# filimonov/ClickHouse

Measured on AMD Instinct MI355X. Metric: rows/sec + achieved HBM GB/s, filter+GROUP-BY on 1 B-row Int64 blocks, 1/2/4/8 GPU, higher is better.
Workload: dtype int64; 1 GPU; BASELINE.json configs[1]: SELECT sum(a), count() WHERE a < 214748365 (~10% pass) over Int64 rows, HBM-resident, fused HIP filter+sum kernel; rows_per_gpu=1000000000, parallelism=single GPU

## Files before the change

### clickhouse_amd/csrc/chgpu_internal.h

```cpp
#pragma once

#include <hip/hip_runtime.h>

#include <cstdarg>
#include <cstdint>
#include <cstdio>
#include <cstring>
#include <map>
#include <string>
#include <type_traits>
#include <vector>

#include "../../include/chgpu.h"

typedef uint64_t u64;
typedef int64_t i64;
typedef uint32_t u32;
typedef int32_t i32;
typedef uint8_t u8;
typedef uint16_t u16;
typedef int16_t i16;
typedef int8_t i8;

int chgpu_set_error(int code, const char * fmt, ...);

#define CHGPU_HIP(expr)                                                                                       \
    do                                                                                                        \
    {                                                                                                         \
        hipError_t _e = (expr);                                                                               \
        if (_e != hipSuccess)                                                                                 \
            return chgpu_set_error(_e == hipErrorOutOfMemory ? CHGPU_ERR_OOM : CHGPU_ERR_DEVICE, "%s: %s (%s:%d)", \
                                   #expr, hipGetErrorString(_e), __FILE__, __LINE__);                        \
    } while (0)

#define CHGPU_TRY(expr)      \
    do                       \
    {                        \
        int _rc = (expr);    \
        if (_rc != CHGPU_OK) \
            return _rc;      \
    } while (0)

#define CHGPU_REQUIRE(cond, code, ...)              \
    do                                              \
    {                                               \
        if (!(cond))                                \
            return chgpu_set_error(code, __VA_ARGS__); \
    } while (0)

static constexpr size_t CHGPU_PAD = 64;

struct chgpu_ctx
{
    int device = 0;
    hipStream_t stream = nullptr;
    bool owns_stream = false;
    int num_cus = 256;
    void * scratch = nullptr;
    size_t scratch_bytes = 0;
    void * pinned = nullptr;
    size_t pinned_bytes = 0;
    hipEvent_t ev_start = nullptr, ev_stop = nullptr;
    u64 counters[CHGPU_N_COUNTERS] = {0};
    u32 * crc_lut_dev = nullptr;
    std::multimap<size_t, void *> pool_free;
    size_t pool_cached_bytes = 0;
    size_t pool_limit_bytes = (size_t)96 << 30;
    long refs = 0;
    bool zombie = false;
    hipStream_t copy_stream = nullptr;
    static constexpr int UPLOAD_RING = 32;
    hipEvent_t upload_done[UPLOAD_RING] = {nullptr};
    hipEvent_t upload_gate = nullptr;
    u64 upload_next_ticket = 1;
    std::map<std::string, long long> options;
};

long long chgpu_opt(const chgpu_ctx * ctx, const char * name, long long dflt);

void chgpu_ctx_retain(chgpu_ctx * ctx);
void chgpu_ctx_release(chgpu_ctx * ctx);

struct chgpu_col
{
    chgpu_ctx * ctx = nullptr;
    int type = 0;
    u64 rows = 0;
    void * data = nullptr;
    void * base = nullptr;
    bool owns = false;
    size_t alloc_bytes = 0;
    int * shared_refs = nullptr;
};

struct ChgpuDeviceGuard
{
    int prev = -1;
    bool switched = false;
    explicit ChgpuDeviceGuard(const chgpu_ctx * ctx)
    {
        if (ctx && hipGetDevice(&prev) == hipSuccess && prev != ctx->device)
            switched = hipSetDevice(ctx->device) == hipSuccess;
    }
    ~ChgpuDeviceGuard()
    {
        if (switched)
            (void)hipSetDevice(prev);
    }
    ChgpuDeviceGuard(const ChgpuDeviceGuard &) = delete;
    ChgpuDeviceGuard & operator=(const ChgpuDeviceGuard &) = delete;
};

static inline size_t chgpu_type_size(int type)
{
    switch (type)
    {
        case CHGPU_I64: case CHGPU_U64: case CHGPU_F64: return 8;
        case CHGPU_U32: case CHGPU_I32: case CHGPU_F32: return 4;
        case CHGPU_U16: case CHGPU_I16: return 2;
        case CHGPU_U8: case CHGPU_I8: return 1;
        default: return 0;
    }
}

static inline bool chgpu_type_is_float(int type) { return type == CHGPU_F64 || type == CHGPU_F32; }
static inline bool chgpu_type_is_int(int type) { return !chgpu_type_is_float(type) && chgpu_type_size(type) != 0; }
static inline bool chgpu_type_is_signed(int type) { return type == CHGPU_I64 || type == CHGPU_I32 || type == CHGPU_I16 || type == CHGPU_I8; }
static inline int chgpu_sum_result_type(int t)
{
    if (chgpu_type_is_float(t)) return CHGPU_F64;
    return chgpu_type_is_signed(t) ? CHGPU_I64 : CHGPU_U64;
}

int chgpu_scratch(chgpu_ctx * ctx, size_t bytes, void ** out);
int chgpu_pool_alloc(chgpu_ctx * ctx, size_t bytes, void ** out, size_t * class_bytes);
void chgpu_pool_free(chgpu_ctx * ctx, void * p, size_t class_bytes);
int chgpu_pinned(chgpu_ctx * ctx, size_t bytes, void ** out);
int chgpu_col_new(chgpu_ctx * ctx, int type, u64 rows, chgpu_col ** out);
int chgpu_read_back(chgpu_ctx * ctx, const void * dev, void * host, size_t bytes);
int chgpu_crc_lut(chgpu_ctx * ctx, const u32 ** lut_dev);

static inline u32 chgpu_grid_for(chgpu_ctx * ctx, u64 work_items, u32 block, u32 blocks_per_cu = 8)
{
    u64 want = (work_items + block - 1) / block;
    u64 cap = (u64)ctx->num_cus * blocks_per_cu;
    if (want < 1) want = 1;
    return (u32)(want < cap ? want : cap);
}

int chgpu_scan_exclusive_u32_u64(chgpu_ctx * ctx, const u32 * in, u64 * out, u64 n, u64 * total_dev, void * tmp, size_t tmp_bytes);
int chgpu_scan_inclusive_u32_u64(chgpu_ctx * ctx, const u32 * in, u64 * out, u64 n, u64 * total_dev, void * tmp, size_t tmp_bytes);
size_t chgpu_scan_tmp_bytes(u64 n);
int chgpu_partition_by_key_byte(chgpu_ctx * ctx, const chgpu_col * keys, u32 shift, u32 n_cols, const chgpu_col * const * cols, chgpu_col ** outs);
int chgpu_partition_core(chgpu_ctx * ctx, const u32 * sel, u64 n, u32 num_shards, u32 n_cols, const chgpu_col * const * cols, chgpu_col ** outs, u64 * counts);
int str_validate_offsets(chgpu_ctx * ctx, const chgpu_col * offsets_u64, const chgpu_col * chars_u8);

template <typename F>
static void dispatch_width(size_t bytes, F && fn)
{
    switch (bytes)
    {
        case 8: return fn(u64{});
        case 4: return fn(u32{});
        case 2: return fn(u16{});
        default: return fn(u8{});
    }
}

template <int LO, int HI, typename F>
static void dispatch_const(u32 v, F && fn)
{
    if constexpr (LO < HI)
        if (v > (u32)LO)
            return dispatch_const<LO + 1, HI>(v, fn);
    fn(std::integral_constant<int, LO>{});
}

template <u32... CODES>
struct OneOf
{
    static bool has(u32 v) { return ((v == CODES) || ...); }
    template <typename F>
    static bool dispatch(u32 v, F && fn)
    {
        return ((v == CODES ? (fn(std::integral_constant<u32, CODES>{}), true) : false) || ...);
    }
};

#ifdef __HIPCC__

static constexpr int WAVE = 64;

__device__ __forceinline__ u32 lane_id() { return __builtin_amdgcn_mbcnt_hi(~0u, __builtin_amdgcn_mbcnt_lo(~0u, 0u)); }

__device__ __forceinline__ u32 mbcnt(u64 mask)
{
    return __builtin_amdgcn_mbcnt_hi((u32)(mask >> 32), __builtin_amdgcn_mbcnt_lo((u32)mask, 0u));
}

__device__ __forceinline__ u64 shfl_down_u64(u64 v, int delta)
{
    u32 lo = __shfl_down((u32)v, delta, WAVE);
    u32 hi = __shfl_down((u32)(v >> 32), delta, WAVE);
    return ((u64)hi << 32) | lo;
}

__device__ __forceinline__ u64 wave_reduce_add_u64(u64 v)
{
#pragma unroll
    for (int d = 32; d >= 1; d >>= 1)
        v += shfl_down_u64(v, d);
    return v;
}

__device__ __forceinline__ double wave_reduce_add_f64(double v)
{
#pragma unroll
    for (int d = 32; d >= 1; d >>= 1)
        v += __longlong_as_double((long long)shfl_down_u64((u64)__double_as_longlong(v), d));
    return v;
}

__device__ __forceinline__ u32 wave_reduce_add_u32(u32 v)
{
#pragma unroll
    for (int d = 32; d >= 1; d >>= 1)
        v += __shfl_down(v, d, WAVE);
    return v;
}

__device__ __forceinline__ u64 wave_reduce_max_u64(u64 v)
{
#pragma unroll
    for (int d = 32; d >= 1; d >>= 1)
    {
        const u64 o = shfl_down_u64(v, d);
        v = o > v ? o : v;
    }
    return v;
}

__device__ __host__ __forceinline__ u64 agg_order_key(u64 bits, int type)
{
    switch (type)
    {
        case CHGPU_I64: case CHGPU_I32: case CHGPU_I16: case CHGPU_I8: return bits ^ 0x8000000000000000ull;
        case CHGPU_F64: case CHGPU_F32: return (bits >> 63) ? ~bits : bits ^ 0x8000000000000000ull;
        default: return bits;
    }
}
__device__ __host__ __forceinline__ u64 agg_order_key_inverse(u64 key, int type)
{
    switch (type)
    {
        case CHGPU_I64: case CHGPU_I32: case CHGPU_I16: case CHGPU_I8: return key ^ 0x8000000000000000ull;
        case CHGPU_F64: case CHGPU_F32: return (key >> 63) ? key ^ 0x8000000000000000ull : ~key;
        default: return key;
    }
}

__device__ __forceinline__ u64 dev_intHash64(u64 x)
{
    x ^= x >> 33;
    x *= 0xff51afd7ed558ccdULL;
    x ^= x >> 33;
    x *= 0xc4ceb9fe1a85ec53ULL;
    x ^= x >> 33;
    return x;
}

__device__ __forceinline__ u32 dev_crc32c_tab(const u32 * __restrict__ lut, u64 x)
{
    u32 r = 0;
#pragma unroll
    for (int j = 0; j < 8; ++j)
        r ^= lut[j * 256 + ((x >> (8 * j)) & 0xFF)];
    return r;
}

__device__ __forceinline__ u32 dev_crc32c_zero8(u32 crc)
{
#pragma unroll 1
    for (int k = 0; k < 64; ++k)
        crc = (crc >> 1) ^ (0x82F63B78u & (0u - (crc & 1u)));
    return crc;
}

#endif
```

### clickhouse_amd/csrc/core.hip

```cpp
#include "chgpu_internal.h"

#include <mutex>

static thread_local char g_last_error[512] = "";

int chgpu_set_error(int code, const char * fmt, ...)
{
    va_list ap;
    va_start(ap, fmt);
    vsnprintf(g_last_error, sizeof(g_last_error), fmt, ap);
    va_end(ap);
    return code;
}

extern "C" const char * chgpu_last_error(void) { return g_last_error; }
extern "C" int chgpu_abi_version(void) { return CHGPU_ABI_VERSION; }

extern "C" int chgpu_ctx_create(int device_id, void * hip_stream, chgpu_ctx ** out)
{
    CHGPU_REQUIRE(out, CHGPU_ERR_BAD_ARGUMENTS, "chgpu_ctx_create: out is NULL");
    int n_dev = 0;
    CHGPU_HIP(hipGetDeviceCount(&n_dev));
    CHGPU_REQUIRE(device_id >= 0 && device_id < n_dev, CHGPU_ERR_BAD_ARGUMENTS, "device %d out of range (%d devices)", device_id, n_dev);
    chgpu_ctx probe_dev;
    probe_dev.device = device_id;
    ChgpuDeviceGuard guard(&probe_dev);
    hipDeviceProp_t prop;
    CHGPU_HIP(hipGetDeviceProperties(&prop, device_id));
    chgpu_ctx * ctx = new chgpu_ctx();
    ctx->device = device_id;
    ctx->num_cus = prop.multiProcessorCount > 0 ? prop.multiProcessorCount : 256;
    if (hip_stream)
    {
        ctx->stream = (hipStream_t)hip_stream;
        ctx->owns_stream = false;
    }
    else
    {
        hipError_t e = hipStreamCreateWithFlags(&ctx->stream, hipStreamNonBlocking);
        if (e != hipSuccess)
        {
            delete ctx;
            return chgpu_set_error(CHGPU_ERR_DEVICE, "hipStreamCreate: %s", hipGetErrorString(e));
        }
        ctx->owns_stream = true;
    }
    (void)hipEventCreate(&ctx->ev_start);
    (void)hipEventCreate(&ctx->ev_stop);
    *out = ctx;
    return CHGPU_OK;
}

static void ctx_teardown(chgpu_ctx * ctx)
{
    ChgpuDeviceGuard guard(ctx);
    (void)hipStreamSynchronize(ctx->stream);
    if (ctx->copy_stream)
    {
        (void)hipStreamSynchronize(ctx->copy_stream);
        (void)hipStreamDestroy(ctx->copy_stream);
    }
    for (auto & e : ctx->upload_done)
        if (e) (void)hipEventDestroy(e);
    if (ctx->upload_gate) (void)hipEventDestroy(ctx->upload_gate);
    if (ctx->scratch) (void)hipFree(ctx->scratch);
    for (auto & kv : ctx->pool_free)
        (void)hipFree(kv.second);
    ctx->pool_free.clear();
    if (ctx->pinned) (void)hipHostFree(ctx->pinned);
    if (ctx->crc_lut_dev) (void)hipFree(ctx->crc_lut_dev);
    if (ctx->ev_start) (void)hipEventDestroy(ctx->ev_start);
    if (ctx->ev_stop) (void)hipEventDestroy(ctx->ev_stop);
    if (ctx->owns_stream) (void)hipStreamDestroy(ctx->stream);
    delete ctx;
}

void chgpu_ctx_retain(chgpu_ctx * ctx)
{
    if (ctx)
        ++ctx->refs;
}

void chgpu_ctx_release(chgpu_ctx * ctx)
{
    if (ctx && --ctx->refs == 0 && ctx->zombie)
        ctx_teardown(ctx);
}

extern "C" int chgpu_ctx_destroy(chgpu_ctx * ctx)
{
    if (!ctx)
        return CHGPU_OK;
    if (ctx->refs > 0)
    {
        ctx->zombie = true;
        return CHGPU_OK;
    }
    ctx_teardown(ctx);
    return CHGPU_OK;
}

extern "C" int chgpu_ctx_synchronize(chgpu_ctx * ctx)
{
    ChgpuDeviceGuard _dev_guard(ctx);
    CHGPU_REQUIRE(ctx, CHGPU_ERR_BAD_ARGUMENTS, "ctx is NULL");
    CHGPU_HIP(hipStreamSynchronize(ctx->stream));
    return CHGPU_OK;
}

static std::mutex g_opt_mu;
static std::map<std::string, long long> g_opt_defaults;
static const char * const CHGPU_OPTION_NAMES[] = {
    "agg_no_partition", "debug", "deterministic_float_sums", "test_chain_grid", "test_group_array_fail_alloc", "test_keydict_chunk_rows", "test_keydict_weak_tags", "test_limit_by_fail_alloc", "test_limit_by_grid", "test_quantile_fail_alloc", "test_quantile_hist_budget",
    "test_string_fail_alloc", "test_uniq_fail_growth",
    "tune_agg_lds_threads", "tune_agg_no_ranged", "tune_agg_ranged_s", "tune_cmp_wg", "tune_expr_wg", "tune_exprn_wg", "tune_fcount_wg",
    "tune_filter_no_multi", "tune_fs2_wg", "tune_fs_wg", "tune_fscatter_wg", "tune_gb_kib", "tune_gb_no_tiled",
    "tune_gb_no_word_passes", "tune_gb_no_two_level", "tune_gb_nocnt32", "tune_gb_noops", "tune_gb_nowide", "tune_gb_s", "tune_gb_tile",
    "tune_gb_unitdiv", "tune_jit_unroll", "tune_jit_wg_map", "tune_jit_wg_sum", "tune_join_cap_shift", "tune_join_eager_build",
    "tune_join_lds_min_rows", "tune_join_no_dense_prefilter", "tune_join_no_fused_payload", "tune_join_no_lds_filter",
    "tune_join_no_lds_probe", "tune_join_no_prefilter", "tune_join_no_dense_map", "tune_join_no_radix",
    "tune_join_no_regions", "tune_join_no_slice_build", "tune_join_region_kib", "tune_join_region_min_rows", "tune_quantile_hist_rounds", "tune_quantile_no_lds_scatter", "tune_str_contains_general",
};

long long chgpu_opt(const chgpu_ctx * ctx, const char * name, long long dflt)
{
    if (ctx && !ctx->options.empty())
    {
        auto it = ctx->options.find(name);
        if (it != ctx->options.end())
            return it->second;
    }
    std::lock_guard<std::mutex> lk(g_opt_mu);
    if (g_opt_defaults.empty())
        return dflt;
    auto it = g_opt_defaults.find(name);
    return it != g_opt_defaults.end() ? it->second : dflt;
}

extern "C" int chgpu_ctx_set_option(chgpu_ctx * ctx, const char * name, int64_t value)
{
    CHGPU_REQUIRE(name, CHGPU_ERR_BAD_ARGUMENTS, "NULL argument");
    bool known = false;
    for (const char * n : CHGPU_OPTION_NAMES)
        known = known || strcmp(n, name) == 0;
    CHGPU_REQUIRE(known, CHGPU_ERR_BAD_ARGUMENTS, "unknown option '%s'", name);
    if (ctx)
        ctx->options[name] = value;
    else
    {
        std::lock_guard<std::mutex> lk(g_opt_mu);
        g_opt_defaults[name] = value;
    }
    return CHGPU_OK;
}

extern "C" int chgpu_ctx_trim(chgpu_ctx * ctx)
{
    ChgpuDeviceGuard _dev_guard(ctx);
    CHGPU_REQUIRE(ctx, CHGPU_ERR_BAD_ARGUMENTS, "ctx is NULL");
    CHGPU_HIP(hipStreamSynchronize(ctx->stream));
    for (auto & kv : ctx->pool_free)
        (void)hipFree(kv.second);
    ctx->pool_free.clear();
    ctx->pool_cached_bytes = 0;
    if (ctx->scratch)
        (void)hipFree(ctx->scratch);
    ctx->scratch = nullptr;
    ctx->scratch_bytes = 0;
    return CHGPU_OK;
}

extern "C" int chgpu_ctx_counters(chgpu_ctx * ctx, uint64_t out[CHGPU_N_COUNTERS])
{
    ChgpuDeviceGuard _dev_guard(ctx);
    CHGPU_REQUIRE(ctx && out, CHGPU_ERR_BAD_ARGUMENTS, "NULL argument");
    memcpy(out, ctx->counters, sizeof(ctx->counters));
    return CHGPU_OK;
}

extern "C" int chgpu_timer_start(chgpu_ctx * ctx)
{
    ChgpuDeviceGuard _dev_guard(ctx);
    CHGPU_REQUIRE(ctx, CHGPU_ERR_BAD_ARGUMENTS, "ctx is NULL");
    CHGPU_HIP(hipEventRecord(ctx->ev_start, ctx->stream));
    return CHGPU_OK;
}

extern "C" int chgpu_timer_stop_ms(chgpu_ctx * ctx, double * elapsed_ms)
{
    ChgpuDeviceGuard _dev_guard(ctx);
    CHGPU_REQUIRE(ctx && elapsed_ms, CHGPU_ERR_BAD_ARGUMENTS, "NULL argument");
    CHGPU_HIP(hipEventRecord(ctx->ev_stop, ctx->stream));
    CHGPU_HIP(hipEventSynchronize(ctx->ev_stop));
    float ms = 0;
    CHGPU_HIP(hipEventElapsedTime(&ms, ctx->ev_start, ctx->ev_stop));
    *elapsed_ms = ms;
    return CHGPU_OK;
}

int chgpu_scratch(chgpu_ctx * ctx, size_t bytes, void ** out)
{
    if (bytes > ctx->scratch_bytes)
    {
        ChgpuDeviceGuard guard(ctx);
        CHGPU_HIP(hipStreamSynchronize(ctx->stream));
        if (ctx->scratch)
            CHGPU_HIP(hipFree(ctx->scratch));
        ctx->scratch = nullptr;
        ctx->scratch_bytes = 0;
        size_t want = bytes + bytes / 4 + (1 << 20);
        CHGPU_HIP(hipMalloc(&ctx->scratch, want));
        ctx->scratch_bytes = want;
    }
    *out = ctx->scratch;
    return CHGPU_OK;
}

int chgpu_pinned(chgpu_ctx * ctx, size_t bytes, void ** out)
{
    if (bytes > ctx->pinned_bytes)
    {
        ChgpuDeviceGuard guard(ctx);
        CHGPU_HIP(hipStreamSynchronize(ctx->stream));
        if (ctx->pinned)
            CHGPU_HIP(hipHostFree(ctx->pinned));
        ctx->pinned = nullptr;
        ctx->pinned_bytes = 0;
        size_t want = bytes < 4096 ? 4096 : bytes;
        CHGPU_HIP(hipHostMalloc(&ctx->pinned, want, hipHostMallocDefault));
        ctx->pinned_bytes = want;
    }
    *out = ctx->pinned;
    return CHGPU_OK;
}

int chgpu_read_back(chgpu_ctx * ctx, const void * dev, void * host, size_t bytes)
{
    void * stage = nullptr;
    CHGPU_TRY(chgpu_pinned(ctx, bytes, &stage));
    CHGPU_HIP(hipMemcpyAsync(stage, dev, bytes, hipMemcpyDeviceToHost, ctx->stream));
    CHGPU_HIP(hipStreamSynchronize(ctx->stream));
    memcpy(host, stage, bytes);
    return CHGPU_OK;
}

static size_t pool_class(size_t bytes)
{
    if (bytes < 4096)
        return 4096;
    size_t p = 4096;
    while (p * 2 <= bytes)
        p *= 2;
    for (int q = 4; q <= 8; ++q)
        if (p / 4 * q >= bytes)
            return p / 4 * q;
    return p * 2;
}

int chgpu_pool_alloc(chgpu_ctx * ctx, size_t bytes, void ** out, size_t * class_bytes)
{
    const size_t cls = pool_class(bytes);
    ChgpuDeviceGuard guard(ctx);
    auto it = ctx->pool_free.lower_bound(cls);
    if (it != ctx->pool_free.end() && it->first <= cls + cls / 2)
    {
        *out = it->second;
        *class_bytes = it->first;
        ctx->pool_cached_bytes -= it->first;
        ctx->pool_free.erase(it);
        return CHGPU_OK;
    }
    hipError_t e = hipMalloc(out, cls);
    if (e == hipErrorOutOfMemory && !ctx->pool_free.empty())
    {
        (void)hipGetLastError();
        (void)hipStreamSynchronize(ctx->stream);
        for (auto & kv : ctx->pool_free)
            (void)hipFree(kv.second);
        ctx->pool_free.clear();
        ctx->pool_cached_bytes = 0;
        e = hipMalloc(out, cls);
    }
    if (e != hipSuccess)
        return chgpu_set_error(e == hipErrorOutOfMemory ? CHGPU_ERR_OOM : CHGPU_ERR_DEVICE, "hipMalloc(%zu): %s", cls, hipGetErrorString(e));
    *class_bytes = cls;
    return CHGPU_OK;
}

void chgpu_pool_free(chgpu_ctx * ctx, void * p, size_t class_bytes)
{
    if (!p)
        return;
    if (ctx->pool_cached_bytes + class_bytes > ctx->pool_limit_bytes)
    {
        (void)hipFree(p);
        return;
    }
    ctx->pool_free.emplace(class_bytes, p);
    ctx->pool_cached_bytes += class_bytes;
}

int chgpu_col_new(chgpu_ctx * ctx, int type, u64 rows, chgpu_col ** out)
{
    size_t es = chgpu_type_size(type);
    CHGPU_REQUIRE(es, CHGPU_ERR_BAD_ARGUMENTS, "unknown column type %d", type);
    ChgpuDeviceGuard guard(ctx);
    size_t bytes = rows * es + 2 * CHGPU_PAD;
    void * base = nullptr;
    size_t cls = 0;
    CHGPU_TRY(chgpu_pool_alloc(ctx, bytes, &base, &cls));
    chgpu_col * c = new chgpu_col();
    chgpu_ctx_retain(ctx);
    c->ctx = ctx;
    c->type = type;
    c->rows = rows;
    c->base = base;
    c->data = (char *)base + CHGPU_PAD;
    c->owns = true;
    c->alloc_bytes = cls;
    *out = c;
    return CHGPU_OK;
}

extern "C" int chgpu_col_alloc(chgpu_ctx * ctx, int type, uint64_t rows, chgpu_col ** out)
{
    ChgpuDeviceGuard _dev_guard(ctx);
    CHGPU_REQUIRE(ctx && out, CHGPU_ERR_BAD_ARGUMENTS, "NULL argument");
    return chgpu_col_new(ctx, type, rows, out);
}

extern "C" int chgpu_col_upload(chgpu_ctx * ctx, int type, const void * host_ptr, uint64_t rows, chgpu_col ** out)
{
    ChgpuDeviceGuard _dev_guard(ctx);
    CHGPU_REQUIRE(ctx && out && (host_ptr || rows == 0), CHGPU_ERR_BAD_ARGUMENTS, "NULL argument");
    chgpu_col * c = nullptr;
    CHGPU_TRY(chgpu_col_new(ctx, type, rows, &c));
    if (rows)
    {
        hipError_t e = hipMemcpyAsync(c->data, host_ptr, rows * chgpu_type_size(type), hipMemcpyHostToDevice, ctx->stream);
        if (e == hipSuccess)
            e = hipStreamSynchronize(ctx->stream);
        if (e != hipSuccess)
        {
            chgpu_col_free(c);
            return chgpu_set_error(CHGPU_ERR_DEVICE, "upload: %s", hipGetErrorString(e));
        }
    }
    *out = c;
    return CHGPU_OK;
}

extern "C" int chgpu_host_alloc(size_t bytes, void ** out)
{
    CHGPU_REQUIRE(out, CHGPU_ERR_BAD_ARGUMENTS, "NULL argument");
    CHGPU_HIP(hipHostMalloc(out, bytes ? bytes : 1, hipHostMallocDefault));
    return CHGPU_OK;
}

extern "C" int chgpu_host_free(void * p)
{
    if (p)
        CHGPU_HIP(hipHostFree(p));
    return CHGPU_OK;
}

extern "C" int chgpu_col_upload_async(chgpu_ctx * ctx, int type, const void * pinned_host_ptr, uint64_t rows, chgpu_col ** out, uint64_t * ticket_out)
{
    CHGPU_REQUIRE(ctx && out && ticket_out && (pinned_host_ptr || rows == 0), CHGPU_ERR_BAD_ARGUMENTS, "NULL argument");
    ChgpuDeviceGuard guard(ctx);
    if (!ctx->copy_stream)
    {
        CHGPU_HIP(hipStreamCreateWithFlags(&ctx->copy_stream, hipStreamNonBlocking));
        CHGPU_HIP(hipEventCreateWithFlags(&ctx->upload_gate, hipEventDisableTiming));
        for (auto & e : ctx->upload_done)
            CHGPU_HIP(hipEventCreateWithFlags(&e, hipEventDisableTiming));
    }
    chgpu_col * c = nullptr;
    CHGPU_TRY(chgpu_col_new(ctx, type, rows, &c));
    const u64 ticket = ctx->upload_next_ticket++;
    hipEvent_t done = ctx->upload_done[ticket % chgpu_ctx::UPLOAD_RING];
    hipError_t e = hipSuccess;
    if ((e = hipEventRecord(ctx->upload_gate, ctx->stream)) == hipSuccess && (e = hipStreamWaitEvent(ctx->copy_stream, ctx->upload_gate, 0)) == hipSuccess)
    {
        if (rows)
            e = hipMemcpyAsync(c->data, pinned_host_ptr, rows * chgpu_type_size(type), hipMemcpyHostToDevice, ctx->copy_stream);
        if (e == hipSuccess)
            e = hipEventRecord(done, ctx->copy_stream);
        if (e == hipSuccess)
            e = hipStreamWaitEvent(ctx->stream, done, 0);
    }
    if (e != hipSuccess)
    {
        chgpu_col_free(c);
        return chgpu_set_error(CHGPU_ERR_DEVICE, "upload_async: %s", hipGetErrorString(e));
    }
    *out = c;
    *ticket_out = ticket;
    return CHGPU_OK;
}

extern "C" int chgpu_upload_wait(chgpu_ctx * ctx, uint64_t ticket)
{
    ChgpuDeviceGuard _dev_guard(ctx);
    CHGPU_REQUIRE(ctx, CHGPU_ERR_BAD_ARGUMENTS, "ctx is NULL");
    if (ticket == 0 || ticket >= ctx->upload_next_ticket)
        return ticket == 0 ? CHGPU_OK : chgpu_set_error(CHGPU_ERR_BAD_ARGUMENTS, "upload ticket %llu was never issued", (unsigned long long)ticket);
    ChgpuDeviceGuard guard(ctx);
    if (ticket + chgpu_ctx::UPLOAD_RING <= ctx->upload_next_ticket)
    {
        CHGPU_HIP(hipStreamSynchronize(ctx->copy_stream));
        return CHGPU_OK;
    }
    CHGPU_HIP(hipEventSynchronize(ctx->upload_done[ticket % chgpu_ctx::UPLOAD_RING]));
    return CHGPU_OK;
}

extern "C" int chgpu_col_wrap(chgpu_ctx * ctx, int type, void * device_ptr, uint64_t rows, chgpu_col ** out)
{
    ChgpuDeviceGuard _dev_guard(ctx);
    CHGPU_REQUIRE(ctx && out && (device_ptr || rows == 0), CHGPU_ERR_BAD_ARGUMENTS, "NULL argument");
    CHGPU_REQUIRE(chgpu_type_size(type), CHGPU_ERR_BAD_ARGUMENTS, "unknown column type %d", type);
    CHGPU_REQUIRE(((uintptr_t)device_ptr % chgpu_type_size(type)) == 0, CHGPU_ERR_BAD_ARGUMENTS, "device pointer not element-aligned");
    chgpu_col * c = new chgpu_col();
    chgpu_ctx_retain(ctx);
    c->ctx = ctx;
    c->type = type;
    c->rows = rows;
    c->data = device_ptr;
    c->owns = false;
    *out = c;
    return CHGPU_OK;
}

extern "C" int chgpu_col_slice(chgpu_ctx * ctx, const chgpu_col * col, uint64_t start, uint64_t rows, chgpu_col ** out)
{
    ChgpuDeviceGuard _dev_guard(ctx);
    CHGPU_REQUIRE(ctx && col && out, CHGPU_ERR_BAD_ARGUMENTS, "NULL argument");
    CHGPU_REQUIRE(start <= col->rows && rows <= col->rows - start, CHGPU_ERR_BAD_ARGUMENTS,
                  "cut(%llu,%llu) out of bounds of a column of %llu rows", (unsigned long long)start, (unsigned long long)rows, (unsigned long long)col->rows);
    return chgpu_col_wrap(ctx, col->type, (char *)col->data + start * chgpu_type_size(col->type), rows, out);
}

extern "C" int chgpu_col_concat(chgpu_ctx * ctx, uint32_t n, const chgpu_col * const * cols, chgpu_col ** out)
{
    ChgpuDeviceGuard _dev_guard(ctx);
    CHGPU_REQUIRE(ctx && cols && out && n >= 1, CHGPU_ERR_BAD_ARGUMENTS, "NULL argument");
    u64 total = 0;
    for (u32 k = 0; k < n; ++k)
    {
        CHGPU_REQUIRE(cols[k], CHGPU_ERR_BAD_ARGUMENTS, "column %u is NULL", k);
        CHGPU_REQUIRE(cols[k]->type == cols[0]->type, CHGPU_ERR_BAD_ARGUMENTS, "columns of different types cannot be concatenated");
        total += cols[k]->rows;
    }
    chgpu_col * r = nullptr;
    CHGPU_TRY(chgpu_col_new(ctx, cols[0]->type, total, &r));
    const size_t es = chgpu_type_size(cols[0]->type);
    u64 pos = 0;
    for (u32 k = 0; k < n; ++k)
    {
        if (cols[k]->rows)
        {
            hipError_t e = hipMemcpyAsync((char *)r->data + pos * es, cols[k]->data, cols[k]->rows * es, hipMemcpyDeviceToDevice, ctx->stream);
            if (e != hipSuccess)
            {
                chgpu_col_free(r);
                return chgpu_set_error(CHGPU_ERR_DEVICE, "concat copy: %s", hipGetErrorString(e));
            }
        }
        pos += cols[k]->rows;
    }
    *out = r;
    return CHGPU_OK;
}

extern "C" int chgpu_col_download(chgpu_ctx * ctx, const chgpu_col * col, void * host_ptr, uint64_t rows)
{
    ChgpuDeviceGuard _dev_guard(ctx);
    CHGPU_REQUIRE(ctx && col && (host_ptr || rows == 0), CHGPU_ERR_BAD_ARGUMENTS, "NULL argument");
    CHGPU_REQUIRE(rows <= col->rows, CHGPU_ERR_SIZES_MISMATCH, "download of %llu rows from a column of %llu", (unsigned long long)rows, (unsigned long long)col->rows);
    if (rows)
    {
        CHGPU_HIP(hipMemcpyAsync(host_ptr, col->data, rows * chgpu_type_size(col->type), hipMemcpyDeviceToHost, ctx->stream));
        CHGPU_HIP(hipStreamSynchronize(ctx->stream));
    }
    return CHGPU_OK;
}

extern "C" int chgpu_col_download_many(chgpu_ctx * ctx, uint32_t n, const chgpu_col * const * cols, void * const * host_ptrs)
{
    ChgpuDeviceGuard _dev_guard(ctx);
    CHGPU_REQUIRE(ctx && (n == 0 || (cols && host_ptrs)), CHGPU_ERR_BAD_ARGUMENTS, "NULL argument");
    bool any = false;
    for (u32 c = 0; c < n; ++c)
    {
        CHGPU_REQUIRE(cols[c] && (host_ptrs[c] || cols[c]->rows == 0), CHGPU_ERR_BAD_ARGUMENTS, "NULL column or host buffer %u", c);
        if (cols[c]->rows)
        {
            CHGPU_HIP(hipMemcpyAsync(host_ptrs[c], cols[c]->data, cols[c]->rows * chgpu_type_size(cols[c]->type), hipMemcpyDeviceToHost, ctx->stream));
            any = true;
        }
    }
    if (any)
        CHGPU_HIP(hipStreamSynchronize(ctx->stream));
    return CHGPU_OK;
}

extern "C" uint64_t chgpu_col_rows(const chgpu_col * col) { return col ? col->rows : 0; }
extern "C" int chgpu_col_type(const chgpu_col * col) { return col ? col->type : -1; }
extern "C" void * chgpu_col_device_ptr(const chgpu_col * col) { return col ? col->data : nullptr; }

extern "C" int chgpu_col_free(chgpu_col * col)
{
    if (!col)
        return CHGPU_OK;
    if (col->owns && col->base)
    {
        bool last = true;
        if (col->shared_refs)
        {
            last = --*col->shared_refs == 0;
            if (last)
                delete col->shared_refs;
        }
        if (last)
        {
            if (col->alloc_bytes && col->ctx)
                chgpu_pool_free(col->ctx, col->base, col->alloc_bytes);
            else
                (void)hipFree(col->base);
        }
    }
    chgpu_ctx * ctx = col->ctx;
    delete col;
    chgpu_ctx_release(ctx);
    return CHGPU_OK;
}

int chgpu_crc_lut(chgpu_ctx * ctx, const u32 ** lut_dev)
{
    if (!ctx->crc_lut_dev)
    {
        ChgpuDeviceGuard guard(ctx);
        std::vector<u32> lut(8 * 256 + 1);
        auto soft = [](u64 x, u32 crc) {
            for (int i = 0; i < 8; ++i)
            {
                crc ^= (u32)((x >> (8 * i)) & 0xFF);
                for (int k = 0; k < 8; ++k)
                    crc = (crc >> 1) ^ (0x82F63B78u & (0u - (crc & 1u)));
            }
            return crc;
        };
        for (int j = 0; j < 8; ++j)
            for (int b = 0; b < 256; ++b)
                lut[j * 256 + b] = soft((u64)b << (8 * j), 0);
        lut[2048] = soft(0, 0xFFFFFFFFu);
        CHGPU_HIP(hipMalloc((void **)&ctx->crc_lut_dev, lut.size() * sizeof(u32)));
        CHGPU_HIP(hipMemcpyAsync(ctx->crc_lut_dev, lut.data(), lut.size() * sizeof(u32), hipMemcpyHostToDevice, ctx->stream));
        CHGPU_HIP(hipStreamSynchronize(ctx->stream));
    }
    *lut_dev = ctx->crc_lut_dev;
    return CHGPU_OK;
}
```

### clickhouse_amd/csrc/expr_jit.hip

```cpp
#include "chgpu_internal.h"

#include <dlfcn.h>

#include <mutex>
#include <string>

namespace
{

struct Rtc
{
    void * h = nullptr;
    int (*create)(void **, const char *, const char *, int, const char * const *, const char * const *) = nullptr;
    int (*compile)(void *, int, const char * const *) = nullptr;
    int (*log_size)(void *, size_t *) = nullptr;
    int (*log)(void *, char *) = nullptr;
    int (*code_size)(void *, size_t *) = nullptr;
    int (*code)(void *, char *) = nullptr;
    int (*destroy)(void **) = nullptr;
};
Rtc g_rtc;
std::mutex g_jit_mutex;
std::map<std::string, std::vector<char>> g_code_cache;
std::map<std::pair<int, std::string>, hipModule_t> g_module_cache;

int rtc_load()
{
    if (g_rtc.h)
        return CHGPU_OK;
    const char * names[] = {"libhiprtc.so.7", "libhiprtc.so", "/opt/rocm/lib/libhiprtc.so"};
    void * h = nullptr;
    for (const char * n : names)
        if ((h = dlopen(n, RTLD_NOW | RTLD_LOCAL)))
            break;
    if (!h)
        return chgpu_set_error(CHGPU_ERR_NOT_IMPLEMENTED, "cannot load libhiprtc (%s): expressions stay on the CPU", dlerror());
#define SYM(field, name)                                              \
    *(void **)&g_rtc.field = dlsym(h, name);                          \
    if (!g_rtc.field)                                                 \
        return chgpu_set_error(CHGPU_ERR_DEVICE, "libhiprtc lacks %s", name);
    SYM(create, "hiprtcCreateProgram")
    SYM(compile, "hiprtcCompileProgram")
    SYM(log_size, "hiprtcGetProgramLogSize")
    SYM(log, "hiprtcGetProgramLog")
    SYM(code_size, "hiprtcGetCodeSize")
    SYM(code, "hiprtcGetCode")
    SYM(destroy, "hiprtcDestroyProgram")
#undef SYM
    g_rtc.h = h;
    return CHGPU_OK;
}

const char * ctype(int t)
{
    switch (t)
    {
        case CHGPU_I64: return "i64";
        case CHGPU_U64: return "u64";
        case CHGPU_I32: return "i32";
        case CHGPU_U32: return "u32";
        case CHGPU_I16: return "i16";
        case CHGPU_U16: return "u16";
        case CHGPU_I8: return "i8";
        case CHGPU_U8: return "u8";
        case CHGPU_F64: return "f64";
        case CHGPU_F32: return "f32";
        default: return nullptr;
    }
}

int construct(bool sgn, bool flt, size_t size)
{
    if (flt)
        return size == 8 ? CHGPU_F64 : size == 4 ? CHGPU_F32 : -1;
    switch (size)
    {
        case 1: return sgn ? CHGPU_I8 : CHGPU_U8;
        case 2: return sgn ? CHGPU_I16 : CHGPU_U16;
        case 4: return sgn ? CHGPU_I32 : CHGPU_U32;
        case 8: return sgn ? CHGPU_I64 : CHGPU_U64;
        default: return -1;
    }
}
size_t next_size(size_t s) { return s < 8 ? s * 2 : s; }
bool is_sgn(int t) { return chgpu_type_is_signed(t) || chgpu_type_is_float(t); }

struct FnRow;
struct Operands
{
    int rt;
    int t[3];
    std::string n[3];
};
typedef int (*TypeRule)(const FnRow & f, int fn, int a, int b, int c);
typedef std::string (*Emitter)(const Operands & x);
typedef const char * (*Gate)(const chgpu_expr_node * nodes, const chgpu_expr_node & nd, const int * at);

struct FnRow
{
    int code, n_codes;
    int arity;
    TypeRule type;
    int result;
    const char * text;
    const char * text_float;
    Emitter emit;
    Gate gate;
};

int ty_fixed(const FnRow & f, int, int a, int b, int)
{
    return chgpu_type_size(a) && (f.arity < 2 || chgpu_type_size(b)) ? f.result : -1;
}
int ty_date(const FnRow & f, int, int a, int, int) { return a == CHGPU_U16 ? f.result : -1; }
bool both_int(int a, int b) { return chgpu_type_is_int(a) && chgpu_type_is_int(b); }
int ty_add_mul(const FnRow &, int, int a, int b, int)
{
    const size_t sa = chgpu_type_size(a), sb = chgpu_type_size(b);
    return (sa && sb) ? construct(is_sgn(a) || is_sgn(b), chgpu_type_is_float(a) || chgpu_type_is_float(b), next_size(sa > sb ? sa : sb)) : -1;
}
int ty_minus(const FnRow &, int, int a, int b, int)
{
    const size_t sa = chgpu_type_size(a), sb = chgpu_type_size(b);
    return (sa && sb) ? construct(true, chgpu_type_is_float(a) || chgpu_type_is_float(b), next_size(sa > sb ? sa : sb)) : -1;
}
int ty_negate(const FnRow &, int, int a, int, int)
{
    const size_t sa = chgpu_type_size(a);
    return sa ? construct(true, chgpu_type_is_float(a), is_sgn(a) ? sa : next_size(sa)) : -1;
}
int ty_bit(const FnRow &, int, int a, int b, int)
{
    return both_int(a, b) ? construct(is_sgn(a) || is_sgn(b), false, std::max(chgpu_type_size(a), chgpu_type_size(b))) : -1;
}
int ty_int_div(const FnRow &, int, int a, int b, int)
{
    return both_int(a, b) ? construct(is_sgn(a) || is_sgn(b), false, chgpu_type_size(a)) : -1;
}
int ty_modulo(const FnRow &, int, int a, int b, int)
{
    return both_int(a, b) ? construct(is_sgn(a), false, is_sgn(a) ? next_size(chgpu_type_size(b)) : chgpu_type_size(b)) : -1;
}
int ty_if(const FnRow &, int, int a, int b, int c)
{
    const size_t sb = chgpu_type_size(b), sc = chgpu_type_size(c);
    if (!chgpu_type_is_int(a) || !sb || !sc)
        return -1;
    if (b == c)
        return b;
    const bool fb = chgpu_type_is_float(b), fc = chgpu_type_is_float(c);
    const bool has_float = fb || fc, has_integer = !fb || !fc, has_signed = is_sgn(b) || is_sgn(c), has_unsigned = !is_sgn(b) || !is_sgn(c);
    const size_t max_u = std::max(is_sgn(b) ? (size_t)0 : sb, is_sgn(c) ? (size_t)0 : sc);
    const size_t max_s = std::max(is_sgn(b) ? sb : (size_t)0, is_sgn(c) ? sc : (size_t)0);
    const size_t max_i = std::max(fb ? (size_t)0 : sb, fc ? (size_t)0 : sc);
    const size_t max_f = std::max(fb ? sb : (size_t)0, fc ? sc : (size_t)0);
    const size_t m = std::max(sb, sc);
    const bool dbl = (has_float && has_integer && max_i >= max_f) || (has_signed && has_unsigned && max_u >= max_s);
    return construct(has_signed, has_float, dbl ? m * 2 : m);
}
int ty_cast(const FnRow & f, int fn, int a, int, int)
{
    const int to = fn - f.code;
    if (!chgpu_type_size(a) || !chgpu_type_size(to))
        return -1;
    if (chgpu_type_is_float(a) && !chgpu_type_is_float(to))
        return -1;
    return to;
}

const char * const NO_SAFE_DIVISOR = "intDiv / modulo need a constant integer divisor that cannot raise ILLEGAL_DIVISION";
bool constant_divisor(const chgpu_expr_node * nodes, const chgpu_expr_node & nd, const int * at, u64 * bits, u64 * mask)
{
    const chgpu_expr_node & dn = nodes[nd.args[1]];
    if (dn.kind != CHGPU_EX_CONST || !both_int(at[0], at[1]))
        return false;
    const size_t sb = chgpu_type_size(at[1]);
    *mask = sb == 8 ? ~0ull : ((1ull << (8 * sb)) - 1);
    *bits = dn.bits & *mask;
    return *bits != 0;
}
const char * gate_int_div(const chgpu_expr_node * nodes, const chgpu_expr_node & nd, const int * at)
{
    u64 bits = 0, mask = 0;
    if (!constant_divisor(nodes, nd, at, &bits, &mask))
        return NO_SAFE_DIVISOR;
    const bool cast_to_signed = chgpu_type_is_signed(at[0]) && chgpu_type_size(at[0]) <= chgpu_type_size(at[1]);
    return bits == mask && (chgpu_type_is_signed(at[1]) || cast_to_signed) ? NO_SAFE_DIVISOR : nullptr;
}
const char * gate_modulo(const chgpu_expr_node * nodes, const chgpu_expr_node & nd, const int * at)
{
    u64 bits = 0, mask = 0;
    if (!constant_divisor(nodes, nd, at, &bits, &mask))
        return NO_SAFE_DIVISOR;
    if (!chgpu_type_is_signed(at[1]))
        return nullptr;
    return bits == mask || bits == (mask >> 1) + 1 ? NO_SAFE_DIVISOR : nullptr;
}

std::string wide(int t, const std::string & e)
{
    if (chgpu_type_is_float(t))
        return "(f64)" + e;
    return (chgpu_type_is_signed(t) ? "(i64)" : "(u64)") + e;
}

std::string subst(const std::string & text, const Operands & x)
{
    std::string s;
    for (size_t i = 0; i < text.size(); ++i)
    {
        if (text[i] != '$')
            s += text[i];
        else if (text[++i] == 'T')
            s += ctype(x.rt);
        else if (text[i] == 'W')
        {
            ++i;
            s += wide(x.t[text[i] - '0'], x.n[text[i] - '0']);
        }
        else
            s += x.n[text[i] - '0'];
    }
    return s;
}

std::string emit_int_div(const Operands & x)
{
    const int ta = x.t[0], tb = x.t[1];
    if (!chgpu_type_is_signed(ta) && !chgpu_type_is_signed(tb))
        return subst("($T)($0 / $1)", x);
    const int sa_t = construct(true, false, chgpu_type_size(ta));
    const int sb_t = chgpu_type_size(ta) <= chgpu_type_size(tb) ? construct(true, false, chgpu_type_size(tb)) : sa_t;
    return subst(std::string("($T)((") + ctype(sa_t) + ")$0 / (" + ctype(sb_t) + ")$1)", x);
}

const FnRow FUNCTIONS[] = {
    {CHGPU_FN_EQUALS, 1, 2, ty_fixed, CHGPU_U8, "(u8)(eq_($W0, $W1))"},
    {CHGPU_FN_NOT_EQUALS, 1, 2, ty_fixed, CHGPU_U8, "(u8)(!eq_($W0, $W1))"},
    {CHGPU_FN_LESS, 1, 2, ty_fixed, CHGPU_U8, "(u8)(lt_($W0, $W1))"},
    {CHGPU_FN_GREATER, 1, 2, ty_fixed, CHGPU_U8, "(u8)(lt_($W1, $W0))"},
    {CHGPU_FN_LESS_OR_EQUALS, 1, 2, ty_fixed, CHGPU_U8, "(u8)(le_($W0, $W1))"},
    {CHGPU_FN_GREATER_OR_EQUALS, 1, 2, ty_fixed, CHGPU_U8, "(u8)(ge_($W0, $W1))"},
    {CHGPU_FN_PLUS, 1, 2, ty_add_mul, -1, "($T)((u64)$0 + (u64)$1)", "(f64)$0 + (f64)$1"},
    {CHGPU_FN_MINUS, 1, 2, ty_minus, -1, "($T)((u64)$0 - (u64)$1)", "(f64)$0 - (f64)$1"},
    {CHGPU_FN_MULTIPLY, 1, 2, ty_add_mul, -1, "($T)((u64)$0 * (u64)$1)", "(f64)$0 * (f64)$1"},
    {CHGPU_FN_DIVIDE, 1, 2, ty_fixed, CHGPU_F64, "(f64)$0 / (f64)$1"},
    {CHGPU_FN_NEGATE, 1, 1, ty_negate, -1, "($T)(0ull - (u64)$0)", "-$0"},
    {CHGPU_FN_INT_DIV, 1, 2, ty_int_div, -1, nullptr, nullptr, emit_int_div, gate_int_div},
    {CHGPU_FN_MODULO, 1, 2, ty_modulo, -1, "($T)($0 % $1)", nullptr, nullptr, gate_modulo},
    {CHGPU_FN_AND, 1, 2, ty_fixed, CHGPU_U8, "(u8)(($0 != 0) & ($1 != 0))"},
    {CHGPU_FN_OR, 1, 2, ty_fixed, CHGPU_U8, "(u8)(($0 != 0) | ($1 != 0))"},
    {CHGPU_FN_XOR, 1, 2, ty_fixed, CHGPU_U8, "(u8)(($0 != 0) ^ ($1 != 0))"},
    {CHGPU_FN_NOT, 1, 1, ty_fixed, CHGPU_U8, "(u8)!($0 != 0)"},
    {CHGPU_FN_IF, 1, 3, ty_if, -1, "($0 != 0) ? ($T)$1 : ($T)$2"},
    {CHGPU_FN_BIT_AND, 1, 2, ty_bit, -1, "($T)((u64)$0 & (u64)$1)"},
    {CHGPU_FN_BIT_OR, 1, 2, ty_bit, -1, "($T)((u64)$0 | (u64)$1)"},
    {CHGPU_FN_BIT_XOR, 1, 2, ty_bit, -1, "($T)((u64)$0 ^ (u64)$1)"},
    {CHGPU_FN_TO_YEAR, 1, 1, ty_date, CHGPU_U16, "(u16)civil_($0).y"},
    {CHGPU_FN_TO_MONTH, 1, 1, ty_date, CHGPU_U8, "(u8)civil_($0).m"},
    {CHGPU_FN_TO_DAY_OF_MONTH, 1, 1, ty_date, CHGPU_U8, "(u8)civil_($0).d"},
    {CHGPU_FN_TO_YYYYMM, 1, 1, ty_date, CHGPU_U32, "(u32)(civil_($0).y * 100u + civil_($0).m)"},
    {CHGPU_FN_TO_YYYYMMDD, 1, 1, ty_date, CHGPU_U32, "(u32)(civil_($0).y * 10000u + civil_($0).m * 100u + civil_($0).d)"},
    {CHGPU_FN_TO_DAY_OF_WEEK, 1, 1, ty_date, CHGPU_U8, "(u8)(((u32)$0 + 3u) % 7u + 1u)"},
    {CHGPU_FN_TO_QUARTER, 1, 1, ty_date, CHGPU_U8, "(u8)((civil_($0).m - 1u) / 3u + 1u)"},
    {CHGPU_FN_TO_START_OF_MONTH, 1, 1, ty_date, CHGPU_U16, "(u16)((u32)$0 - (civil_($0).d - 1u))"},
    {CHGPU_FN_CAST, 16, 1, ty_cast, -1, "($T)$0"},
};

const FnRow * fn_row(int fn)
{
    for (const FnRow & f : FUNCTIONS)
        if (fn >= f.code && fn < f.code + f.n_codes)
            return &f;
    return nullptr;
}

const char * PRELUDE = R"SRC(
typedef unsigned long long u64; typedef long long i64; typedef unsigned int u32; typedef int i32;
typedef unsigned short u16; typedef short i16; typedef unsigned char u8; typedef signed char i8;
typedef float f32; typedef double f64;
#define DEV static __device__ __forceinline__
// accurate::lessOp / equalsOp (AccurateComparison.h:20-204) on operands widened to i64 / u64 / f64: mathematically exact
DEV bool nan_(i64) { return false; }
DEV bool nan_(u64) { return false; }
DEV bool nan_(f64 x) { return x != x; }
DEV bool lt_(i64 a, i64 b) { return a < b; }
DEV bool lt_(u64 a, u64 b) { return a < b; }
DEV bool lt_(f64 a, f64 b) { return a < b; }
DEV bool lt_(i64 a, u64 b) { return a < 0 || (u64)a < b; }
DEV bool lt_(u64 a, i64 b) { return b >= 0 && a < (u64)b; }
DEV bool lt_(i64 a, f64 b)
{
    if (b != b) return false;
    if (b >= 9223372036854775808.0) return true;
    if (b < -9223372036854775808.0) return false;
    const i64 t = (i64)b; // truncation, exact in range
    if (a != t) return a < t;
    return b - (f64)t > 0;
}
DEV bool lt_(f64 a, i64 b)
{
    if (a != a) return false;
    if (a >= 9223372036854775808.0) return false;
    if (a < -9223372036854775808.0) return true;
    const i64 t = (i64)a;
    if (t != b) return t < b;
    return a - (f64)t < 0;
}
DEV bool lt_(u64 a, f64 b)
{
    if (b != b) return false;
    if (b >= 18446744073709551616.0) return true;
    if (b <= 0) return false;
    const u64 t = (u64)b;
    if (a != t) return a < t;
    return b - (f64)t > 0;
}
DEV bool lt_(f64 a, u64 b)
{
    if (a != a) return false;
    if (a >= 18446744073709551616.0) return false;
    if (a < 0) return true;
    const u64 t = (u64)a;
    if (t != b) return t < b;
    return a - (f64)t < 0;
}
DEV bool eq_(i64 a, i64 b) { return a == b; }
DEV bool eq_(u64 a, u64 b) { return a == b; }
DEV bool eq_(f64 a, f64 b) { return a == b; }
DEV bool eq_(i64 a, u64 b) { return a >= 0 && (u64)a == b; }
DEV bool eq_(u64 a, i64 b) { return b >= 0 && a == (u64)b; }
DEV bool eq_(i64 a, f64 b)
{
    if (!(b >= -9223372036854775808.0 && b < 9223372036854775808.0)) return false;
    const i64 t = (i64)b;
    return t == a && (f64)t == b;
}
DEV bool eq_(f64 a, i64 b) { return eq_(b, a); }
DEV bool eq_(u64 a, f64 b)
{
    if (!(b >= 0 && b < 18446744073709551616.0)) return false;
    const u64 t = (u64)b;
    return t == a && (f64)t == b;
}
DEV bool eq_(f64 a, u64 b) { return eq_(b, a); }
template <typename A, typename B> DEV bool le_(A a, B b) { return !nan_(a) && !nan_(b) && !lt_(b, a); }
template <typename A, typename B> DEV bool ge_(A a, B b) { return !nan_(a) && !nan_(b) && !lt_(a, b); }
// DayNum -> civil date (proleptic Gregorian; what DateLUTImpl's day table holds for DayNum, Common/DateLUTImpl.h)
struct Civil { u32 y, m, d; };
DEV Civil civil_(u32 days)
{
    const u32 z = days + 719468u;
    const u32 era = z / 146097u;
    const u32 doe = z - era * 146097u;
    const u32 yoe = (doe - doe / 1460u + doe / 36524u - doe / 146096u) / 365u;
    const u32 doy = doe - (365u * yoe + yoe / 4u - yoe / 100u);
    const u32 mp = (5u * doy + 2u) / 153u;
    Civil c;
    c.d = doy - (153u * mp + 2u) / 5u + 1u;
    c.m = mp < 10u ? mp + 3u : mp - 9u;
    c.y = yoe + era * 400u + (c.m <= 2u ? 1u : 0u);
    return c;
}
)SRC";

}

struct chgpu_expr
{
    std::vector<chgpu_expr_node> nodes;
    std::vector<int> types;
    std::vector<int> input_types;
    std::string body;
};


namespace
{

int build_body(chgpu_expr * e)
{
    std::string s;
    char buf[256];
    for (size_t k = 0; k < e->nodes.size(); ++k)
    {
        const chgpu_expr_node & nd = e->nodes[k];
        const int t = e->types[k];
        const char * ct = ctype(t);
        std::string rhs;
        if (nd.kind == CHGPU_EX_INPUT)
            rhs = "r.c" + std::to_string(nd.code);
        else if (nd.kind == CHGPU_EX_CONST)
        {
            if (t == CHGPU_F64)
                snprintf(buf, sizeof(buf), "__longlong_as_double((long long)0x%llxull)", (unsigned long long)nd.bits);
            else if (t == CHGPU_F32)
                snprintf(buf, sizeof(buf), "__uint_as_float(0x%xu)", (unsigned)(nd.bits & 0xffffffffu));
            else
                snprintf(buf, sizeof(buf), "(%s)0x%llxull", ct, (unsigned long long)nd.bits);
            rhs = buf;
        }
        else
        {
            const FnRow & f = *fn_row(nd.code);
            Operands x;
            x.rt = t;
            for (int j = 0; j < f.arity; ++j)
            {
                x.t[j] = e->types[nd.args[j]];
                x.n[j] = "n" + std::to_string(nd.args[j]);
            }
            rhs = f.emit ? f.emit(x) : subst(f.text_float && chgpu_type_is_float(t) ? f.text_float : f.text, x);
        }
        s += std::string("    const ") + ct + " n" + std::to_string(k) + " = " + rhs + ";\n";
    }
    e->body = s;
    return CHGPU_OK;
}

u32 vec_rows(const std::vector<int> & types)
{
    size_t wmax = 1, wmin = 8;
    for (int t : types)
    {
        const size_t w = chgpu_type_size(t);
        wmax = std::max(wmax, w);
        wmin = std::min(wmin, w);
    }
    u32 v = (u32)std::max((size_t)16 / wmax, (size_t)4 / wmin);
    return v < 1 ? 1 : v > 16 ? 16 : v;
}

enum Form
{
    FORM_MAP,
    FORM_SUM,
    FORM_WHERE_MAP,
};

struct KernelSpec
{
    Form form = FORM_MAP;
    std::vector<u32> out_nodes;
    int filter_node = -1;
    int value_node = -1;
    u32 vec = 1;
};

static int jit_env(const chgpu_ctx * ctx, const char * name, int dflt) { return (int)chgpu_opt(ctx, name, dflt); }
static int jit_unroll()
{
    static const int v = jit_env(nullptr, "tune_jit_unroll", 4);
    return v;
}
#define JIT_UNROLL jit_unroll()
constexpr u32 JIT_MAX_COLS = 8;

struct JitArgs
{
    const void * in[JIT_MAX_COLS];
    void * out[JIT_MAX_COLS];
    u64 n;
    u64 * part;
    u32 n_parts;
    u32 pad;
};
const char * const ARGS_DECL = "struct Args { const void * in[8]; void * out[8]; u64 n; u64 * part; u32 n_parts; u32 pad; };\n";
static_assert(JIT_MAX_COLS == 8 && sizeof(JitArgs) == 2 * 8 * 8 + 8 + 8 + 4 + 4, "ARGS_DECL restates JitArgs");

struct ResField
{
    std::string type, name, value;
};

std::vector<ResField> out_fields(const chgpu_expr * e, const std::vector<u32> & out_nodes)
{
    std::vector<ResField> fields;
    for (size_t o = 0; o < out_nodes.size(); ++o)
        fields.push_back({ctype(e->types[out_nodes[o]]), "o" + std::to_string(o), "n" + std::to_string(out_nodes[o])});
    return fields;
}

std::string gen_frame(const chgpu_expr * e, const std::string & decls, bool keep, int filter_node, const std::vector<ResField> & fields)
{
    std::string s = PRELUDE + decls + ARGS_DECL + "struct Row {";
    for (size_t j = 0; j < e->input_types.size(); ++j)
        if (e->input_types[j] >= 0)
            s += std::string(" ") + ctype(e->input_types[j]) + " c" + std::to_string(j) + ";";
    s += " };\nstruct Res {";
    if (keep)
        s += " bool keep;";
    for (const ResField & f : fields)
        s += " " + f.type + " " + f.name + ";";
    s += " };\nDEV void eval(const Row & r, Res & o)\n{\n" + e->body;
    if (keep)
        s += filter_node >= 0 ? "    o.keep = n" + std::to_string(filter_node) + " != 0;\n" : std::string("    o.keep = true;\n");
    for (const ResField & f : fields)
        s += "    o." + f.name + " = " + f.value + ";\n";
    return s + "}\n";
}

std::string row_load(const chgpu_expr * e, const std::string & indent, const std::string & index)
{
    std::string s;
    for (size_t j = 0; j < e->input_types.size(); ++j)
        if (e->input_types[j] >= 0)
            s += indent + "r.c" + std::to_string(j) + " = ((const " + ctype(e->input_types[j]) + " *)a.in[" + std::to_string(j) + "])[" + index + "];\n";
    return s;
}

std::string out_store(const std::string & indent, const std::string & type, size_t o, const std::string & index, const std::string & value)
{
    return indent + "((" + type + " *)a.out[" + std::to_string(o) + "])[" + index + "] = " + value + ";\n";
}

std::string gen_source(const chgpu_expr * e, const KernelSpec & ks)
{
    const bool fsum = ks.form == FORM_SUM;
    const u32 V = ks.vec;
    auto vtype = [&](int t) { return std::string("v") + ctype(t) + "_t"; };
    auto otype = [&](size_t o) { return e->types[ks.out_nodes[o]]; };
    const size_t n_out = ks.out_nodes.size();
    std::string vdefs;
    for (int t = 0; t <= CHGPU_F32; ++t)
        vdefs += std::string("typedef ") + ctype(t) + " " + vtype(t) + " __attribute__((ext_vector_type(" + std::to_string(V) + ")));\n";
    std::vector<ResField> fields = out_fields(e, ks.out_nodes);
    if (fsum && ks.value_node >= 0)
        fields.push_back({ctype(e->types[ks.value_node]), "val", "n" + std::to_string(ks.value_node)});
    std::string s = gen_frame(e, vdefs, fsum, ks.filter_node, fields);

    const bool facc = fsum && ks.value_node >= 0 && chgpu_type_is_float(e->types[ks.value_node]);
    auto accumulate = [&](const std::string & indent) {
        std::string t;
        if (ks.value_node >= 0)
            t += indent + (facc ? "acc += o.keep ? (f64)o.val : 0.0;\n" : "acc += o.keep ? (u64)o.val : 0ull;\n");
        return t + indent + "cnt += o.keep ? 1u : 0u;\n";
    };
    const std::string U = std::to_string(JIT_UNROLL), VS = std::to_string(V);
    s += "extern \"C\" __global__ __launch_bounds__(256) void k_run(Args a)\n{\n";
    if (fsum)
        s += facc ? "    f64 acc = 0; u64 cnt = 0;\n" : "    u64 acc = 0; u64 cnt = 0;\n";
    s += "    const u64 nvec = a.n / " + VS + ";\n    constexpr u64 CH = 256ull * " + U + ";\n    const u64 nch = nvec / CH;\n";
    const bool tr_ok = !fsum && V * (u32)JIT_UNROLL == 16;
    std::vector<int> tr_slot(n_out, -1);
    int n_tr = 0;
    if (tr_ok)
        for (size_t o = 0; o < n_out; ++o)
            if (chgpu_type_size(otype(o)) == 1)
                tr_slot[o] = n_tr++;
    if (n_tr)
        s += "    typedef u8 v16b_t __attribute__((ext_vector_type(16)));\n    __shared__ __attribute__((aligned(16))) u8 tr[" + std::to_string(n_tr) + "][4][1024];\n";
    s += "    for (u64 ch = blockIdx.x; ch < nch; ch += gridDim.x)\n    {\n        const u64 sb = ch * CH + (u64)(threadIdx.x >> 6) * (64 * " + U +
         ");\n        const u64 vb = sb + (threadIdx.x & 63);\n";
    for (size_t j = 0; j < e->input_types.size(); ++j)
        if (e->input_types[j] >= 0)
        {
            const std::string vt = vtype(e->input_types[j]), J = std::to_string(j);
            s += "        " + vt + " x" + J + "[" + U + "];\n";
            s += "#pragma unroll\n        for (int k = 0; k < " + U + "; ++k) x" + J + "[k] = __builtin_nontemporal_load((const " + vt + " *)a.in[" + J + "] + vb + (u64)k * 64);\n";
        }
    s += "#pragma unroll\n        for (int k = 0; k < " + U + "; ++k)\n        {\n";
    for (size_t o = 0; o < n_out; ++o)
        s += "            " + vtype(otype(o)) + " y" + std::to_string(o) + ";\n";
    s += "#pragma unroll\n            for (int q = 0; q < " + VS + "; ++q)\n            {\n                Row r; Res o;\n";
    for (size_t j = 0; j < e->input_types.size(); ++j)
        if (e->input_types[j] >= 0)
            s += "                r.c" + std::to_string(j) + " = x" + std::to_string(j) + "[k][q];\n";
    s += "                eval(r, o);\n";
    if (fsum)
        s += accumulate("                ");
    for (size_t o = 0; o < n_out; ++o)
        s += "                y" + std::to_string(o) + "[q] = o.o" + std::to_string(o) + ";\n";
    s += "            }\n";
    for (size_t o = 0; o < n_out; ++o)
    {
        if (tr_slot[o] >= 0)
            s += "            *(" + vtype(otype(o)) + " *)&tr[" + std::to_string(tr_slot[o]) + "][threadIdx.x >> 6][(k * 64 + (threadIdx.x & 63)) * " + VS +
                 "] = y" + std::to_string(o) + ";\n";
        else
            s += out_store("            ", vtype(otype(o)), o, "vb + (u64)k * 64", "y" + std::to_string(o));
    }
    s += "        }\n";
    if (n_tr)
    {
        s += "        __builtin_amdgcn_wave_barrier();\n";
        for (size_t o = 0; o < n_out; ++o)
            if (tr_slot[o] >= 0)
                s += "        *((v16b_t *)((u8 *)a.out[" + std::to_string(o) + "] + sb * " + VS + ") + (threadIdx.x & 63)) = *(const v16b_t *)&tr[" +
                     std::to_string(tr_slot[o]) + "][threadIdx.x >> 6][(threadIdx.x & 63) * 16];\n";
        s += "        __builtin_amdgcn_wave_barrier();\n";
    }
    s += "    }\n";
    s += "    for (u64 i = nch * CH * " + VS + " + (u64)blockIdx.x * 256 + threadIdx.x; i < a.n; i += (u64)gridDim.x * 256)\n    {\n        Row r; Res o;\n";
    s += row_load(e, "        ", "i") + "        eval(r, o);\n";
    if (fsum)
        s += accumulate("        ");
    for (size_t o = 0; o < n_out; ++o)
        s += out_store("        ", ctype(otype(o)), o, "i", "o.o" + std::to_string(o));
    s += "    }\n";
    if (fsum)
    {
        s += R"SRC(
    __shared__ u64 sh_a[4], sh_c[4];
    u64 ab = ACC_BITS(acc);
#pragma unroll
    for (int d = 32; d >= 1; d >>= 1)
    {
        const u64 oa = ((u64)__shfl_down((u32)(ab >> 32), d, 64) << 32) | __shfl_down((u32)ab, d, 64);
        const u64 oc = ((u64)__shfl_down((u32)(cnt >> 32), d, 64) << 32) | __shfl_down((u32)cnt, d, 64);
        ab = ACC_ADD(ab, oa);
        cnt += oc;
    }
    if ((threadIdx.x & 63) == 0) { sh_a[threadIdx.x >> 6] = ab; sh_c[threadIdx.x >> 6] = cnt; }
    __syncthreads();
    if (threadIdx.x == 0)
    {
        u64 ta = sh_a[0], tc = sh_c[0];
        for (int w = 1; w < 4; ++w) { ta = ACC_ADD(ta, sh_a[w]); tc += sh_c[w]; }
        a.part[2 * blockIdx.x] = ta;
        a.part[2 * blockIdx.x + 1] = tc;
    }
}
extern "C" __global__ __launch_bounds__(64) void k_fin(Args a)
{
    if (threadIdx.x != 0) return;
    u64 ta = ACC_ZERO, tc = 0;
    for (u32 p = 0; p < a.n_parts; ++p) { ta = ACC_ADD(ta, a.part[2 * p]); tc += a.part[2 * p + 1]; }
    a.part[2 * a.n_parts] = ta;
    a.part[2 * a.n_parts + 1] = tc;
}
)SRC";
        const std::string defs = facc ? "#define ACC_BITS(x) ((u64)__double_as_longlong(x))\n#define ACC_ADD(x, y) ((u64)__double_as_longlong(__longlong_as_double((long long)(x)) + __longlong_as_double((long long)(y))))\n#define ACC_ZERO 0ull\n"
                                      : "#define ACC_BITS(x) (x)\n#define ACC_ADD(x, y) ((x) + (y))\n#define ACC_ZERO 0ull\n";
        s = defs + s;
    }
    else
        s += "}\n";
    return s;
}

constexpr u32 FE_CHUNK = 1024;

std::string gen_filter_source(const chgpu_expr * e, const KernelSpec & ks)
{
    std::string s = gen_frame(e, "", true, ks.filter_node, out_fields(e, ks.out_nodes));
    const std::string load = row_load(e, "            ", "in ? i : 0");
    const std::string C = std::to_string(FE_CHUNK);
    s += "extern \"C\" __global__ __launch_bounds__(256) void k_fcount(Args a)\n{\n"
         "    const u32 lane = threadIdx.x & 63;\n"
         "    const u64 n_chunks = (a.n + " + C + " - 1) / " + C + ";\n"
         "    for (u64 ch = ((u64)blockIdx.x * 256 + threadIdx.x) >> 6; ch < n_chunks; ch += ((u64)gridDim.x * 256) >> 6)\n    {\n"
         "        u32 cnt = 0;\n"
         "#pragma unroll 4\n"
         "        for (u32 st = 0; st < " + C + " / 64; ++st)\n        {\n"
         "            const u64 i = ch * " + C + " + st * 64 + lane;\n            const bool in = i < a.n;\n            Row r; Res o;\n" + load +
         "            eval(r, o);\n            cnt += (u32)__popcll(__ballot(in && o.keep));\n        }\n"
         "        if (lane == 0) ((u32 *)a.part)[ch] = cnt;\n    }\n}\n";
    s += "extern \"C\" __global__ __launch_bounds__(256) void k_femit(Args a)\n{\n"
         "    const u32 lane = threadIdx.x & 63;\n"
         "    const u64 n_chunks = (a.n + " + C + " - 1) / " + C + ";\n"
         "    const u64 * offsets = (const u64 *)a.part;\n"
         "    for (u64 ch = ((u64)blockIdx.x * 256 + threadIdx.x) >> 6; ch < n_chunks; ch += ((u64)gridDim.x * 256) >> 6)\n    {\n"
         "        u64 pos = offsets[ch];\n"
         "#pragma unroll 4\n"
         "        for (u32 st = 0; st < " + C + " / 64; ++st)\n        {\n"
         "            const u64 i = ch * " + C + " + st * 64 + lane;\n            const bool in = i < a.n;\n            Row r; Res o;\n" + load +
         "            eval(r, o);\n            const bool keep = in && o.keep;\n            const u64 b = __ballot(keep);\n"
         "            const u64 dst = pos + __builtin_amdgcn_mbcnt_hi((u32)(b >> 32), __builtin_amdgcn_mbcnt_lo((u32)b, 0u));\n"
         "            if (keep)\n            {\n";
    for (size_t o = 0; o < ks.out_nodes.size(); ++o)
        s += out_store("                ", ctype(e->types[ks.out_nodes[o]]), o, "dst", "o.o" + std::to_string(o));
    s += "            }\n            pos += (u64)__popcll(b);\n        }\n    }\n}\n";
    return s;
}

std::string gen_minmax_source(const chgpu_expr * e, int filter_node, int value_node)
{
    const std::string v = "n" + std::to_string(value_node);
    const std::string key = chgpu_type_is_signed(e->types[value_node]) ? "(u64)(i64)" + v + " ^ 0x8000000000000000ull" : "(u64)" + v;
    std::string s = gen_frame(e, "", true, filter_node, {{"u64", "key", key}});
    s += R"SRC(
DEV u64 shfl_u64(u64 v, int d) { return ((u64)__shfl_down((u32)(v >> 32), d, 64) << 32) | __shfl_down((u32)v, d, 64); }
extern "C" __global__ __launch_bounds__(256) void k_mm(Args a)
{
    u64 lo = ~0ull, hi = 0ull, cnt = 0;
    const u64 stride = (u64)gridDim.x * 256;
    for (u64 i0 = (u64)blockIdx.x * 256 + threadIdx.x; i0 < a.n; i0 += stride * 4)
    {
#pragma unroll
        for (int q = 0; q < 4; ++q)
        {
            const u64 i = i0 + (u64)q * stride;
            const bool in = i < a.n;
            Row r; Res o;
)SRC" + row_load(e, "            ", "in ? i : 0") + R"SRC(
            eval(r, o);
            if (in && o.keep) { lo = o.key < lo ? o.key : lo; hi = o.key > hi ? o.key : hi; ++cnt; }
        }
    }
#pragma unroll
    for (int d = 32; d >= 1; d >>= 1)
    {
        const u64 l2 = shfl_u64(lo, d), h2 = shfl_u64(hi, d), c2 = shfl_u64(cnt, d);
        lo = l2 < lo ? l2 : lo; hi = h2 > hi ? h2 : hi; cnt += c2;
    }
    __shared__ u64 sl[4], sh[4], sc[4];
    if ((threadIdx.x & 63) == 0) { sl[threadIdx.x >> 6] = lo; sh[threadIdx.x >> 6] = hi; sc[threadIdx.x >> 6] = cnt; }
    __syncthreads();
    if (threadIdx.x == 0)
    {
        for (int w = 1; w < 4; ++w) { lo = sl[w] < lo ? sl[w] : lo; hi = sh[w] > hi ? sh[w] : hi; cnt += sc[w]; }
        a.part[3 * blockIdx.x] = lo; a.part[3 * blockIdx.x + 1] = hi; a.part[3 * blockIdx.x + 2] = cnt;
    }
}
extern "C" __global__ __launch_bounds__(64) void k_mm_fin(Args a)
{
    if (threadIdx.x != 0) return;
    u64 lo = ~0ull, hi = 0ull, cnt = 0;
    for (u32 p = 0; p < a.n_parts; ++p)
    {
        const u64 l2 = a.part[3 * p], h2 = a.part[3 * p + 1];
        lo = l2 < lo ? l2 : lo; hi = h2 > hi ? h2 : hi; cnt += a.part[3 * p + 2];
    }
    a.part[3 * a.n_parts] = lo; a.part[3 * a.n_parts + 1] = hi; a.part[3 * a.n_parts + 2] = cnt;
}
)SRC";
    return s;
}

int jit_compile(const std::string & src, const std::vector<char> ** code_out)
{
    std::lock_guard<std::mutex> g(g_jit_mutex);
    auto it = g_code_cache.find(src);
    if (it == g_code_cache.end())
    {
        CHGPU_TRY(rtc_load());
        void * prog = nullptr;
        if (g_rtc.create(&prog, src.c_str(), "chgpu_expr.hip", 0, nullptr, nullptr) != 0)
            return chgpu_set_error(CHGPU_ERR_DEVICE, "hiprtcCreateProgram failed");
        const char * opts[] = {"--offload-arch=gfx950", "-O3", "-ffp-contract=off"};
        const int rc = g_rtc.compile(prog, 3, opts);
        if (rc != 0)
        {
            size_t ls = 0;
            g_rtc.log_size(prog, &ls);
            std::string log(ls + 1, '\0');
            if (ls)
                g_rtc.log(prog, &log[0]);
            g_rtc.destroy(&prog);
            if (getenv("CHGPU_JIT_DUMP"))
                fprintf(stderr, "%s\n", src.c_str());
            return chgpu_set_error(CHGPU_ERR_LOGICAL, "hiprtc compile failed (%d): %.400s", rc, log.c_str());
        }
        size_t cs = 0;
        g_rtc.code_size(prog, &cs);
        std::vector<char> code(cs);
        g_rtc.code(prog, code.data());
        g_rtc.destroy(&prog);
        it = g_code_cache.emplace(src, std::move(code)).first;
    }
    *code_out = &it->second;
    return CHGPU_OK;
}

int jit_module(chgpu_ctx * ctx, const std::string & src, hipModule_t * mod)
{
    const std::vector<char> * code = nullptr;
    CHGPU_TRY(jit_compile(src, &code));
    std::lock_guard<std::mutex> g(g_jit_mutex);
    auto key = std::make_pair(ctx->device, src);
    auto it = g_module_cache.find(key);
    if (it == g_module_cache.end())
    {
        hipModule_t m = nullptr;
        CHGPU_HIP(hipModuleLoadData(&m, code->data()));
        it = g_module_cache.emplace(key, m).first;
    }
    *mod = it->second;
    return CHGPU_OK;
}

int check_spec(const chgpu_expr * e, uint32_t n_cols, const chgpu_col * const * cols, u64 * rows_out)
{
    CHGPU_REQUIRE(n_cols >= e->input_types.size(), CHGPU_ERR_BAD_ARGUMENTS, "expression reads column %zu, %u columns given", e->input_types.size() - 1, n_cols);
    u64 rows = 0;
    bool first = true;
    for (size_t j = 0; j < e->input_types.size(); ++j)
    {
        if (e->input_types[j] < 0)
            continue;
        CHGPU_REQUIRE(cols[j], CHGPU_ERR_BAD_ARGUMENTS, "column %zu is NULL", j);
        CHGPU_REQUIRE(cols[j]->type == e->input_types[j], CHGPU_ERR_BAD_ARGUMENTS, "column %zu has type %d, the expression was compiled for %d", j, cols[j]->type, e->input_types[j]);
        if (first)
            rows = cols[j]->rows, first = false;
        CHGPU_REQUIRE(cols[j]->rows == rows, CHGPU_ERR_SIZES_MISMATCH, "Sizes of columns doesn't match: %llu and %llu", (unsigned long long)cols[j]->rows, (unsigned long long)rows);
    }
    CHGPU_REQUIRE(!first, CHGPU_ERR_BAD_ARGUMENTS, "an expression without input columns has no row count");
    *rows_out = rows;
    return CHGPU_OK;
}

int check_filter_node(const chgpu_expr * e, int filter_node, bool required)
{
    CHGPU_REQUIRE(filter_node < (int)e->types.size() && (filter_node >= 0 || !required), CHGPU_ERR_BAD_ARGUMENTS, "bad node");
    CHGPU_REQUIRE(filter_node < 0 || chgpu_type_is_int(e->types[filter_node]), CHGPU_ERR_BAD_ARGUMENTS,
                  "Illegal type for filter: the WHERE node must be an integer (FilterDescription.cpp:86-92)");
    return CHGPU_OK;
}

int make_spec(const chgpu_expr * e, Form form, uint32_t n_outputs, const uint32_t * out_nodes, int filter_node, int value_node, bool aligned, KernelSpec * ks)
{
    ks->form = form;
    std::vector<int> touched;
    for (int t : e->input_types)
        if (t >= 0)
            touched.push_back(t);
    if (form == FORM_SUM)
    {
        CHGPU_REQUIRE(value_node < (int)e->types.size(), CHGPU_ERR_BAD_ARGUMENTS, "bad node");
        ks->value_node = value_node;
    }
    else
    {
        const uint32_t most = form == FORM_WHERE_MAP ? JIT_MAX_COLS - 1 : JIT_MAX_COLS;
        CHGPU_REQUIRE(n_outputs > 0 && n_outputs <= most && out_nodes, CHGPU_ERR_BAD_ARGUMENTS, "1..%u outputs", most);
        for (uint32_t o = 0; o < n_outputs; ++o)
        {
            CHGPU_REQUIRE(out_nodes[o] < e->types.size(), CHGPU_ERR_BAD_ARGUMENTS, "bad output node");
            ks->out_nodes.push_back(out_nodes[o]);
            touched.push_back(e->types[out_nodes[o]]);
        }
    }
    if (form != FORM_MAP)
    {
        CHGPU_TRY(check_filter_node(e, filter_node, form == FORM_WHERE_MAP));
        ks->filter_node = filter_node;
    }
    ks->vec = aligned ? vec_rows(touched) : 1;
    return CHGPU_OK;
}

bool cols_aligned(const chgpu_expr * e, const chgpu_col * const * cols)
{
    for (size_t j = 0; j < e->input_types.size(); ++j)
        if (e->input_types[j] >= 0 && ((uintptr_t)cols[j]->data & 63) != 0)
            return false;
    return true;
}

JitArgs bind_inputs(const chgpu_expr * e, const chgpu_col * const * cols, u64 rows)
{
    JitArgs a;
    memset(&a, 0, sizeof(a));
    for (size_t j = 0; j < e->input_types.size(); ++j)
        a.in[j] = e->input_types[j] >= 0 ? cols[j]->data : nullptr;
    a.n = rows;
    return a;
}

struct NamedFn
{
    const char * name;
    hipFunction_t * fn;
};
int jit_functions(chgpu_ctx * ctx, const std::string & src, std::initializer_list<NamedFn> fns)
{
    hipModule_t mod = nullptr;
    CHGPU_TRY(jit_module(ctx, src, &mod));
    for (const NamedFn & f : fns)
        CHGPU_HIP(hipModuleGetFunction(f.fn, mod, f.name));
    return CHGPU_OK;
}

int launch(chgpu_ctx * ctx, hipFunction_t fn, u32 grid, u32 block, JitArgs & a)
{
    void * params[] = {&a};
    CHGPU_HIP(hipModuleLaunchKernel(fn, grid, 1, 1, block, 1, 1, 0, ctx->stream, params, nullptr));
    return CHGPU_OK;
}

u64 run_items(u64 rows, const KernelSpec & ks)
{
    return (rows + ks.vec * JIT_UNROLL - 1) / (ks.vec * JIT_UNROLL);
}

int run_reduction(chgpu_ctx * ctx, const chgpu_expr * e, const chgpu_col * const * cols, u64 rows, const std::string & src, const char * kernel,
                  const char * fin, u64 items, int wg_per_cu, u32 words, u64 * res)
{
    hipFunction_t fn = nullptr, ffin = nullptr;
    CHGPU_TRY(jit_functions(ctx, src, {{kernel, &fn}, {fin, &ffin}}));
    const u32 grid = chgpu_grid_for(ctx, items, 256, wg_per_cu);
    void * scratch = nullptr;
    CHGPU_TRY(chgpu_scratch(ctx, ((size_t)grid + 1) * words * sizeof(u64), &scratch));
    JitArgs a = bind_inputs(e, cols, rows);
    a.part = (u64 *)scratch;
    a.n_parts = grid;
    CHGPU_TRY(launch(ctx, fn, grid, 256, a));
    CHGPU_TRY(launch(ctx, ffin, 1, 64, a));
    ctx->counters[6] += 2;
    return chgpu_read_back(ctx, a.part + (size_t)words * grid, res, words * sizeof(u64));
}

struct OutCols
{
    std::vector<chgpu_col *> cols;
    ~OutCols()
    {
        for (chgpu_col * c : cols)
            chgpu_col_free(c);
    }
    int alloc(chgpu_ctx * ctx, const chgpu_expr * e, const std::vector<u32> & out_nodes, u64 rows, JitArgs & a)
    {
        for (size_t o = 0; o < out_nodes.size(); ++o)
        {
            chgpu_col * c = nullptr;
            CHGPU_TRY(chgpu_col_new(ctx, e->types[out_nodes[o]], rows, &c));
            cols.push_back(c);
            a.out[o] = c->data;
        }
        return CHGPU_OK;
    }
    void hand_over(chgpu_col ** outs)
    {
        std::copy(cols.begin(), cols.end(), outs);
        cols.clear();
    }
};

}

extern "C" int chgpu_expr_compile(uint32_t n_nodes, const chgpu_expr_node * nodes, chgpu_expr ** out)
{
    CHGPU_REQUIRE(nodes && out && n_nodes > 0, CHGPU_ERR_BAD_ARGUMENTS, "NULL argument");
    CHGPU_REQUIRE(n_nodes <= 256, CHGPU_ERR_NOT_IMPLEMENTED, "expression of %u nodes", n_nodes);
    chgpu_expr * e = new chgpu_expr;
    e->nodes.assign(nodes, nodes + n_nodes);
    e->types.assign(n_nodes, -1);
    int rc = CHGPU_OK;
    for (uint32_t k = 0; k < n_nodes && rc == CHGPU_OK; ++k)
    {
        const chgpu_expr_node & nd = nodes[k];
        if (nd.kind == CHGPU_EX_INPUT)
        {
            if (nd.code < 0 || (u32)nd.code >= JIT_MAX_COLS || !chgpu_type_size(nd.type))
                rc = chgpu_set_error(CHGPU_ERR_BAD_ARGUMENTS, "node %u: input column %d of type %d", k, nd.code, nd.type);
            else
            {
                if (e->input_types.size() <= (size_t)nd.code)
                    e->input_types.resize(nd.code + 1, -1);
                if (e->input_types[nd.code] >= 0 && e->input_types[nd.code] != nd.type)
                    rc = chgpu_set_error(CHGPU_ERR_BAD_ARGUMENTS, "node %u: column %d declared with two types", k, nd.code);
                e->input_types[nd.code] = nd.type;
                e->types[k] = nd.type;
            }
        }
        else if (nd.kind == CHGPU_EX_CONST)
        {
            if (!chgpu_type_size(nd.type))
                rc = chgpu_set_error(CHGPU_ERR_BAD_ARGUMENTS, "node %u: constant of type %d", k, nd.type);
            e->types[k] = nd.type;
        }
        else if (nd.kind == CHGPU_EX_FUNC)
        {
            const FnRow * f = fn_row(nd.code);
            const int ar = f ? f->arity : 2;
            int at[3] = {-1, -1, -1};
            for (int j = 0; j < ar && rc == CHGPU_OK; ++j)
            {
                if (nd.args[j] < 0 || (u32)nd.args[j] >= k)
                    rc = chgpu_set_error(CHGPU_ERR_BAD_ARGUMENTS, "node %u: operand %d is not an earlier node", k, j);
                else
                    at[j] = e->types[nd.args[j]];
            }
            if (rc == CHGPU_OK && f && f->gate)
                if (const char * why_not = f->gate(nodes, nd, at))
                    rc = chgpu_set_error(CHGPU_ERR_NOT_IMPLEMENTED, "node %u: %s", k, why_not);
            if (rc == CHGPU_OK)
            {
                e->types[k] = f ? f->type(*f, nd.code, at[0], at[1], at[2]) : -1;
                if (e->types[k] < 0)
                    rc = chgpu_set_error(CHGPU_ERR_NOT_IMPLEMENTED, "node %u: function %d over types (%d, %d, %d)", k, nd.code, at[0], at[1], at[2]);
            }
        }
        else
            rc = chgpu_set_error(CHGPU_ERR_BAD_ARGUMENTS, "node %u: kind %d", k, nd.kind);
    }
    if (rc == CHGPU_OK)
        rc = build_body(e);
    if (rc != CHGPU_OK)
    {
        delete e;
        return rc;
    }
    *out = e;
    return CHGPU_OK;
}

extern "C" int chgpu_expr_node_type(const chgpu_expr * e, uint32_t node, int * type_out)
{
    CHGPU_REQUIRE(e && type_out && node < e->types.size(), CHGPU_ERR_BAD_ARGUMENTS, "bad node");
    *type_out = e->types[node];
    return CHGPU_OK;
}

extern "C" int chgpu_expr_free(chgpu_expr * e)
{
    delete e;
    return CHGPU_OK;
}

extern "C" int chgpu_expr_precompile(const chgpu_expr * e, uint32_t n_outputs, const uint32_t * out_nodes, int filter_node, int value_node,
                                     uint64_t * code_bytes_out)
{
    CHGPU_REQUIRE(e, CHGPU_ERR_BAD_ARGUMENTS, "NULL argument");
    KernelSpec ks;
    CHGPU_TRY(make_spec(e, n_outputs == 0 ? FORM_SUM : filter_node >= 0 ? FORM_WHERE_MAP : FORM_MAP, n_outputs, out_nodes, filter_node, value_node, true, &ks));
    const std::vector<char> * code = nullptr;
    CHGPU_TRY(jit_compile(ks.form == FORM_WHERE_MAP ? gen_filter_source(e, ks) : gen_source(e, ks), &code));
    if (code_bytes_out)
        *code_bytes_out = code->size();
    return CHGPU_OK;
}

extern "C" int chgpu_expr_execute(chgpu_ctx * ctx, const chgpu_expr * e, uint32_t n_cols, const chgpu_col * const * cols, uint32_t n_outputs,
                                  const uint32_t * out_nodes, chgpu_col ** outs)
{
    ChgpuDeviceGuard _dev_guard(ctx);
    CHGPU_REQUIRE(ctx && e && cols && outs, CHGPU_ERR_BAD_ARGUMENTS, "NULL argument");
    u64 rows = 0;
    CHGPU_TRY(check_spec(e, n_cols, cols, &rows));
    KernelSpec ks;
    CHGPU_TRY(make_spec(e, FORM_MAP, n_outputs, out_nodes, -1, -1, cols_aligned(e, cols), &ks));
    hipFunction_t fn = nullptr;
    CHGPU_TRY(jit_functions(ctx, gen_source(e, ks), {{"k_run", &fn}}));
    JitArgs a = bind_inputs(e, cols, rows);
    OutCols res;
    CHGPU_TRY(res.alloc(ctx, e, ks.out_nodes, rows, a));
    if (rows)
    {
        CHGPU_TRY(launch(ctx, fn, chgpu_grid_for(ctx, run_items(rows, ks), 256, jit_env(ctx, "tune_jit_wg_map", 4)), 256, a));
        ctx->counters[6] += 1;
    }
    res.hand_over(outs);
    return CHGPU_OK;
}

extern "C" int chgpu_expr_filter_sum_node(chgpu_ctx * ctx, const chgpu_expr * e, uint32_t n_cols, const chgpu_col * const * cols, int filter_node,
                                          int value_node, int * result_type_out, void * sum_out, uint64_t * count_out)
{
    ChgpuDeviceGuard _dev_guard(ctx);
    CHGPU_REQUIRE(ctx && e && cols, CHGPU_ERR_BAD_ARGUMENTS, "NULL argument");
    u64 rows = 0;
    CHGPU_TRY(check_spec(e, n_cols, cols, &rows));
    KernelSpec ks;
    CHGPU_TRY(make_spec(e, FORM_SUM, 0, nullptr, filter_node, value_node, cols_aligned(e, cols), &ks));
    if (result_type_out)
        *result_type_out = value_node >= 0 ? chgpu_sum_result_type(e->types[value_node]) : CHGPU_U64;
    u64 res[2] = {0, 0};
    if (rows)
        CHGPU_TRY(run_reduction(ctx, e, cols, rows, gen_source(e, ks), "k_run", "k_fin", run_items(rows, ks), jit_env(ctx, "tune_jit_wg_sum", 2), 2, res));
    if (sum_out)
        memcpy(sum_out, &res[0], 8);
    if (count_out)
        *count_out = res[1];
    return CHGPU_OK;
}

extern "C" int chgpu_expr_filter_execute(chgpu_ctx * ctx, const chgpu_expr * e, uint32_t n_cols, const chgpu_col * const * cols, uint32_t filter_node,
                                         uint32_t n_outputs, const uint32_t * out_nodes, chgpu_col ** outs, uint64_t * rows_out)
{
    ChgpuDeviceGuard _dev_guard(ctx);
    CHGPU_REQUIRE(ctx && e && cols && outs && rows_out && out_nodes, CHGPU_ERR_BAD_ARGUMENTS, "NULL argument");
    KernelSpec ks;
    CHGPU_TRY(make_spec(e, FORM_WHERE_MAP, n_outputs, out_nodes, (int)filter_node, -1, false, &ks));
    u64 rows = 0;
    CHGPU_TRY(check_spec(e, n_cols, cols, &rows));
    JitArgs a = bind_inputs(e, cols, rows);
    OutCols res;
    u64 total = 0;
    if (rows)
    {
        hipFunction_t fcount = nullptr, femit = nullptr;
        CHGPU_TRY(jit_functions(ctx, gen_filter_source(e, ks), {{"k_fcount", &fcount}, {"k_femit", &femit}}));
        const u64 n_chunks = (rows + FE_CHUNK - 1) / FE_CHUNK;
        auto al = [](size_t b) { return (b + 255) / 256 * 256; };
        const size_t b_cnt = al(n_chunks * 4), b_off = al(n_chunks * 8), b_tmp = chgpu_scan_tmp_bytes(n_chunks);
        void * scratch = nullptr;
        CHGPU_TRY(chgpu_scratch(ctx, b_cnt + b_off + 256 + b_tmp, &scratch));
        u32 * counts = (u32 *)scratch;
        u64 * offsets = (u64 *)((char *)scratch + b_cnt);
        u64 * total_dev = (u64 *)((char *)scratch + b_cnt + b_off);
        void * tmp = (char *)scratch + b_cnt + b_off + 256;
        a.part = (u64 *)counts;
        const u32 grid = chgpu_grid_for(ctx, n_chunks * 64, 256, 8);
        CHGPU_TRY(launch(ctx, fcount, grid, 256, a));
        CHGPU_TRY(chgpu_scan_exclusive_u32_u64(ctx, counts, offsets, n_chunks, total_dev, tmp, b_tmp));
        CHGPU_TRY(chgpu_read_back(ctx, total_dev, &total, sizeof(total)));
        CHGPU_TRY(res.alloc(ctx, e, ks.out_nodes, total, a));
        if (total)
        {
            a.part = offsets;
            CHGPU_TRY(launch(ctx, femit, grid, 256, a));
        }
        ctx->counters[6] += 2;
        ctx->counters[0] += total;
    }
    else
        CHGPU_TRY(res.alloc(ctx, e, ks.out_nodes, 0, a));
    res.hand_over(outs);
    *rows_out = total;
    return CHGPU_OK;
}

extern "C" int chgpu_expr_filter_minmax_node(chgpu_ctx * ctx, const chgpu_expr * e, uint32_t n_cols, const chgpu_col * const * cols, int filter_node,
                                             uint32_t value_node, int * value_type_out, void * min_out, void * max_out, uint64_t * count_out)
{
    ChgpuDeviceGuard _dev_guard(ctx);
    CHGPU_REQUIRE(ctx && e && cols, CHGPU_ERR_BAD_ARGUMENTS, "NULL argument");
    CHGPU_REQUIRE(value_node < e->types.size(), CHGPU_ERR_BAD_ARGUMENTS, "bad node");
    CHGPU_TRY(check_filter_node(e, filter_node, false));
    const int vt = e->types[value_node];
    CHGPU_REQUIRE(chgpu_type_is_int(vt), CHGPU_ERR_NOT_IMPLEMENTED,
                  "min / max of a Float column keep a NaN that arrives first (SingleValueDataFixed::setIfSmaller): order-dependent, CPU path");
    u64 rows = 0;
    CHGPU_TRY(check_spec(e, n_cols, cols, &rows));
    if (value_type_out)
        *value_type_out = vt;
    u64 res[3] = {~0ull, 0, 0};
    if (rows)
        CHGPU_TRY(run_reduction(ctx, e, cols, rows, gen_minmax_source(e, filter_node, (int)value_node), "k_mm", "k_mm_fin", (rows + 3) / 4, 8, 3, res));
    const u64 sign = chgpu_type_is_signed(vt) ? 0x8000000000000000ull : 0;
    const u64 vmin = res[2] ? (res[0] ^ sign) : 0, vmax = res[2] ? (res[1] ^ sign) : 0;
    const size_t es = chgpu_type_size(vt);
    if (min_out)
        memcpy(min_out, &vmin, es);
    if (max_out)
        memcpy(max_out, &vmax, es);
    if (count_out)
        *count_out = res[2];
    return CHGPU_OK;
}
```

Baseline: 894.2 billion rows/s.

## Add lazy value-column loading for filtered sums and prune dead expression nodes

```diff
diff --git a/clickhouse_amd/csrc/chgpu_internal.h b/clickhouse_amd/csrc/chgpu_internal.h
--- a/clickhouse_amd/csrc/chgpu_internal.h
+++ b/clickhouse_amd/csrc/chgpu_internal.h
@@ -74,6 +74,7 @@
     hipEvent_t upload_gate = nullptr;
     u64 upload_next_ticket = 1;
     std::map<std::string, long long> options;
+    std::map<std::string, double> jit_pass_rate;
 };
 
 long long chgpu_opt(const chgpu_ctx * ctx, const char * name, long long dflt);
diff --git a/clickhouse_amd/csrc/core.hip b/clickhouse_amd/csrc/core.hip
--- a/clickhouse_amd/csrc/core.hip
+++ b/clickhouse_amd/csrc/core.hip
@@ -116,7 +116,7 @@
     "tune_agg_lds_threads", "tune_agg_no_ranged", "tune_agg_ranged_s", "tune_cmp_wg", "tune_expr_wg", "tune_exprn_wg", "tune_fcount_wg",
     "tune_filter_no_multi", "tune_fs2_wg", "tune_fs_wg", "tune_fscatter_wg", "tune_gb_kib", "tune_gb_no_tiled",
     "tune_gb_no_word_passes", "tune_gb_no_two_level", "tune_gb_nocnt32", "tune_gb_noops", "tune_gb_nowide", "tune_gb_s", "tune_gb_tile",
-    "tune_gb_unitdiv", "tune_jit_unroll", "tune_jit_wg_map", "tune_jit_wg_sum", "tune_join_cap_shift", "tune_join_eager_build",
+    "tune_gb_unitdiv", "tune_jit_lazy", "tune_jit_unroll", "tune_jit_wg_map", "tune_jit_wg_sum", "tune_join_cap_shift", "tune_join_eager_build",
     "tune_join_lds_min_rows", "tune_join_no_dense_prefilter", "tune_join_no_fused_payload", "tune_join_no_lds_filter",
     "tune_join_no_lds_probe", "tune_join_no_prefilter", "tune_join_no_dense_map", "tune_join_no_radix",
     "tune_join_no_regions", "tune_join_no_slice_build", "tune_join_region_kib", "tune_join_region_min_rows", "tune_quantile_hist_rounds", "tune_quantile_no_lds_scatter", "tune_str_contains_general",
diff --git a/clickhouse_amd/csrc/expr_jit.hip b/clickhouse_amd/csrc/expr_jit.hip
--- a/clickhouse_amd/csrc/expr_jit.hip
+++ b/clickhouse_amd/csrc/expr_jit.hip
@@ -2,6 +2,7 @@
 
 #include <dlfcn.h>
 
+#include <cmath>
 #include <mutex>
 #include <string>
 
@@ -371,7 +372,7 @@
     std::vector<chgpu_expr_node> nodes;
     std::vector<int> types;
     std::vector<int> input_types;
-    std::string body;
+    std::vector<std::string> stmts;
 };
 
 
@@ -380,7 +381,6 @@
 
 int build_body(chgpu_expr * e)
 {
-    std::string s;
     char buf[256];
     for (size_t k = 0; k < e->nodes.size(); ++k)
     {
@@ -412,10 +412,49 @@
             }
             rhs = f.emit ? f.emit(x) : subst(f.text_float && chgpu_type_is_float(t) ? f.text_float : f.text, x);
         }
-        s += std::string("    const ") + ct + " n" + std::to_string(k) + " = " + rhs + ";\n";
-    }
-    e->body = s;
-    return CHGPU_OK;
+        e->stmts.push_back(std::string("    const ") + ct + " n" + std::to_string(k) + " = " + rhs + ";\n");
+    }
+    return CHGPU_OK;
+}
+
+struct Deps
+{
+    std::vector<char> node, col;
+};
+Deps closure(const chgpu_expr * e, const std::vector<int> & roots)
+{
+    Deps d{std::vector<char>(e->nodes.size(), 0), std::vector<char>(e->input_types.size(), 0)};
+    for (int r : roots)
+        if (r >= 0 && (size_t)r < d.node.size())
+            d.node[r] = 1;
+    for (size_t k = e->nodes.size(); k-- > 0;)
+    {
+        if (!d.node[k])
+            continue;
+        const chgpu_expr_node & nd = e->nodes[k];
+        if (nd.kind == CHGPU_EX_INPUT)
+            d.col[nd.code] = 1;
+        else if (nd.kind == CHGPU_EX_FUNC)
+            for (int j = 0; j < fn_row(nd.code)->arity; ++j)
+                d.node[nd.args[j]] = 1;
+    }
+    return d;
+}
+Deps operator|(Deps a, const Deps & b)
+{
+    for (size_t k = 0; k < a.node.size(); ++k)
+        a.node[k] |= b.node[k];
+    for (size_t j = 0; j < a.col.size(); ++j)
+        a.col[j] |= b.col[j];
+    return a;
+}
+std::string statements(const chgpu_expr * e, const Deps & d)
+{
+    std::string s;
+    for (size_t k = 0; k < e->stmts.size(); ++k)
+        if (d.node[k])
+            s += e->stmts[k];
+    return s;
 }
 
 u32 vec_rows(const std::vector<int> & types)
@@ -445,6 +484,11 @@
     int filter_node = -1;
     int value_node = -1;
     u32 vec = 1;
+    Deps live;
+    Deps filter, value;
+    bool lazy = false;
+    bool filter_col(size_t j) const { return filter.col[j]; }
+    bool value_only(size_t j) const { return value.col[j] && !filter.col[j]; }
 };
 
 static int jit_env(const chgpu_ctx * ctx, const char * name, int dflt) { return (int)chgpu_opt(ctx, name, dflt); }
@@ -481,18 +525,18 @@
     return fields;
 }
 
-std::string gen_frame(const chgpu_expr * e, const std::string & decls, bool keep, int filter_node, const std::vector<ResField> & fields)
+std::string gen_frame(const chgpu_expr * e, const Deps & live, const std::string & decls, bool keep, int filter_node, const std::vector<ResField> & fields)
 {
     std::string s = PRELUDE + decls + ARGS_DECL + "struct Row {";
-    for (size_t j = 0; j < e->input_types.size(); ++j)
-        if (e->input_types[j] >= 0)
+    for (size_t j = 0; j < live.col.size(); ++j)
+        if (live.col[j])
             s += std::string(" ") + ctype(e->input_types[j]) + " c" + std::to_string(j) + ";";
     s += " };\nstruct Res {";
     if (keep)
         s += " bool keep;";
     for (const ResField & f : fields)
         s += " " + f.type + " " + f.name + ";";
-    s += " };\nDEV void eval(const Row & r, Res & o)\n{\n" + e->body;
+    s += " };\nDEV void eval(const Row & r, Res & o)\n{\n" + statements(e, live);
     if (keep)
         s += filter_node >= 0 ? "    o.keep = n" + std::to_string(filter_node) + " != 0;\n" : std::string("    o.keep = true;\n");
     for (const ResField & f : fields)
@@ -500,11 +544,11 @@
     return s + "}\n";
 }
 
-std::string row_load(const chgpu_expr * e, const std::string & indent, const std::string & index)
+std::string row_load(const chgpu_expr * e, const std::vector<char> & which, const std::string & indent, const std::string & index)
 {
     std::string s;
-    for (size_t j = 0; j < e->input_types.size(); ++j)
-        if (e->input_types[j] >= 0)
+    for (size_t j = 0; j < which.size(); ++j)
+        if (which[j])
             s += indent + "r.c" + std::to_string(j) + " = ((const " + ctype(e->input_types[j]) + " *)a.in[" + std::to_string(j) + "])[" + index + "];\n";
     return s;
 }
@@ -512,6 +556,58 @@
 std::string out_store(const std::string & indent, const std::string & type, size_t o, const std::string & index, const std::string & value)
 {
     return indent + "((" + type + " *)a.out[" + std::to_string(o) + "])[" + index + "] = " + value + ";\n";
+}
+
+constexpr u32 FIN_THREADS = 256;
+std::string sum_finish(const std::string & kernel, bool facc)
+{
+    const std::string defs = facc ? "#define ACC_BITS(x) ((u64)__double_as_longlong(x))\n#define ACC_ADD(x, y) ((u64)__double_as_longlong(__longlong_as_double((long long)(x)) + __longlong_as_double((long long)(y))))\n#define ACC_ZERO 0ull\n"
+                                  : "#define ACC_BITS(x) (x)\n#define ACC_ADD(x, y) ((x) + (y))\n#define ACC_ZERO 0ull\n";
+    return defs + kernel + R"SRC(
+    __shared__ u64 sh_a[4], sh_c[4];
+    u64 ab = ACC_BITS(acc);
+#pragma unroll
+    for (int d = 32; d >= 1; d >>= 1)
+    {
+        const u64 oa = ((u64)__shfl_down((u32)(ab >> 32), d, 64) << 32) | __shfl_down((u32)ab, d, 64);
+        const u64 oc = ((u64)__shfl_down((u32)(cnt >> 32), d, 64) << 32) | __shfl_down((u32)cnt, d, 64);
+        ab = ACC_ADD(ab, oa);
+        cnt += oc;
+    }
+    if ((threadIdx.x & 63) == 0) { sh_a[threadIdx.x >> 6] = ab; sh_c[threadIdx.x >> 6] = cnt; }
+    __syncthreads();
+    if (threadIdx.x == 0)
+    {
+        u64 ta = sh_a[0], tc = sh_c[0];
+        for (int w = 1; w < 4; ++w) { ta = ACC_ADD(ta, sh_a[w]); tc += sh_c[w]; }
+        a.part[2 * blockIdx.x] = ta;
+        a.part[2 * blockIdx.x + 1] = tc;
+    }
+}
+extern "C" __global__ __launch_bounds__(256) void k_fin(Args a)
+{
+    constexpr u32 BATCH = 2048; // partials per turn: 8 workgroups per CU on 256 CUs, 32 KiB
+    __shared__ u64 sh[2 * BATCH];
+    u64 ta = ACC_ZERO, tc = 0;
+    for (u32 p0 = 0; p0 < a.n_parts; p0 += BATCH)
+    {
+        const u32 m = a.n_parts - p0 < BATCH ? a.n_parts - p0 : BATCH;
+        for (u32 i = threadIdx.x; i < 2 * m; i += 256) sh[i] = a.part[2 * (u64)p0 + i];
+        __syncthreads();
+        if (threadIdx.x == 0)
+        {
+#pragma unroll 8
+            for (u32 p = 0; p < m; ++p) { ta = ACC_ADD(ta, sh[2 * p]); tc += sh[2 * p + 1]; }
+        }
+        __syncthreads();
+    }
+    if (threadIdx.x == 0)
+    {
+        a.part[2 * a.n_parts] = ta;
+        a.part[2 * a.n_parts + 1] = tc;
+    }
+}
+)SRC";
 }
 
 std::string gen_source(const chgpu_expr * e, const KernelSpec & ks)
@@ -527,7 +623,7 @@
     std::vector<ResField> fields = out_fields(e, ks.out_nodes);
     if (fsum && ks.value_node >= 0)
         fields.push_back({ctype(e->types[ks.value_node]), "val", "n" + std::to_string(ks.value_node)});
-    std::string s = gen_frame(e, vdefs, fsum, ks.filter_node, fields);
+    std::string s = gen_frame(e, ks.live, vdefs, fsum, ks.filter_node, fields);
 
     const bool facc = fsum && ks.value_node >= 0 && chgpu_type_is_float(e->types[ks.value_node]);
     auto accumulate = [&](const std::string & indent) {
@@ -552,8 +648,8 @@
         s += "    typedef u8 v16b_t __attribute__((ext_vector_type(16)));\n    __shared__ __attribute__((aligned(16))) u8 tr[" + std::to_string(n_tr) + "][4][1024];\n";
     s += "    for (u64 ch = blockIdx.x; ch < nch; ch += gridDim.x)\n    {\n        const u64 sb = ch * CH + (u64)(threadIdx.x >> 6) * (64 * " + U +
          ");\n        const u64 vb = sb + (threadIdx.x & 63);\n";
-    for (size_t j = 0; j < e->input_types.size(); ++j)
-        if (e->input_types[j] >= 0)
+    for (size_t j = 0; j < ks.live.col.size(); ++j)
+        if (ks.live.col[j])
         {
             const std::string vt = vtype(e->input_types[j]), J = std::to_string(j);
             s += "        " + vt + " x" + J + "[" + U + "];\n";
@@ -563,8 +659,8 @@
     for (size_t o = 0; o < n_out; ++o)
         s += "            " + vtype(otype(o)) + " y" + std::to_string(o) + ";\n";
     s += "#pragma unroll\n            for (int q = 0; q < " + VS + "; ++q)\n            {\n                Row r; Res o;\n";
-    for (size_t j = 0; j < e->input_types.size(); ++j)
-        if (e->input_types[j] >= 0)
+    for (size_t j = 0; j < ks.live.col.size(); ++j)
+        if (ks.live.col[j])
             s += "                r.c" + std::to_string(j) + " = x" + std::to_string(j) + "[k][q];\n";
     s += "                eval(r, o);\n";
     if (fsum)
@@ -592,59 +688,80 @@
     }
     s += "    }\n";
     s += "    for (u64 i = nch * CH * " + VS + " + (u64)blockIdx.x * 256 + threadIdx.x; i < a.n; i += (u64)gridDim.x * 256)\n    {\n        Row r; Res o;\n";
-    s += row_load(e, "        ", "i") + "        eval(r, o);\n";
+    s += row_load(e, ks.live.col, "        ", "i") + "        eval(r, o);\n";
     if (fsum)
         s += accumulate("        ");
     for (size_t o = 0; o < n_out; ++o)
         s += out_store("        ", ctype(otype(o)), o, "i", "o.o" + std::to_string(o));
     s += "    }\n";
-    if (fsum)
-    {
-        s += R"SRC(
-    __shared__ u64 sh_a[4], sh_c[4];
-    u64 ab = ACC_BITS(acc);
-#pragma unroll
-    for (int d = 32; d >= 1; d >>= 1)
-    {
-        const u64 oa = ((u64)__shfl_down((u32)(ab >> 32), d, 64) << 32) | __shfl_down((u32)ab, d, 64);
-        const u64 oc = ((u64)__shfl_down((u32)(cnt >> 32), d, 64) << 32) | __shfl_down((u32)cnt, d, 64);
-        ab = ACC_ADD(ab, oa);
-        cnt += oc;
-    }
-    if ((threadIdx.x & 63) == 0) { sh_a[threadIdx.x >> 6] = ab; sh_c[threadIdx.x >> 6] = cnt; }
-    __syncthreads();
-    if (threadIdx.x == 0)
-    {
-        u64 ta = sh_a[0], tc = sh_c[0];
-        for (int w = 1; w < 4; ++w) { ta = ACC_ADD(ta, sh_a[w]); tc += sh_c[w]; }
-        a.part[2 * blockIdx.x] = ta;
-        a.part[2 * blockIdx.x + 1] = tc;
-    }
-}
-extern "C" __global__ __launch_bounds__(64) void k_fin(Args a)
-{
-    if (threadIdx.x != 0) return;
-    u64 ta = ACC_ZERO, tc = 0;
-    for (u32 p = 0; p < a.n_parts; ++p) { ta = ACC_ADD(ta, a.part[2 * p]); tc += a.part[2 * p + 1]; }
-    a.part[2 * a.n_parts] = ta;
-    a.part[2 * a.n_parts + 1] = tc;
-}
-)SRC";
-        const std::string defs = facc ? "#define ACC_BITS(x) ((u64)__double_as_longlong(x))\n#define ACC_ADD(x, y) ((u64)__double_as_longlong(__longlong_as_double((long long)(x)) + __longlong_as_double((long long)(y))))\n#define ACC_ZERO 0ull\n"
-                                      : "#define ACC_BITS(x) (x)\n#define ACC_ADD(x, y) ((x) + (y))\n#define ACC_ZERO 0ull\n";
-        s = defs + s;
-    }
-    else
-        s += "}\n";
-    return s;
+    return fsum ? sum_finish(s, facc) : s + "}\n";
+}
+
+std::string gen_lazy_sum_source(const chgpu_expr * e, const KernelSpec & ks)
+{
+    const u32 V = ks.vec;
+    auto vtype = [&](int t) { return std::string("v") + ctype(t) + "_t"; };
+    std::string vdefs;
+    for (int t = 0; t <= CHGPU_F32; ++t)
+        vdefs += std::string("typedef ") + ctype(t) + " " + vtype(t) + " __attribute__((ext_vector_type(" + std::to_string(V) + ")));\n";
+    const std::string vt = ctype(e->types[ks.value_node]);
+    std::string s = gen_frame(e, ks.live, vdefs, false, -1, {});
+    s += "DEV bool eval_keep(const Row & r)\n{\n" + statements(e, ks.filter) + "    return n" + std::to_string(ks.filter_node) + " != 0;\n}\n";
+    s += "DEV " + vt + " eval_val(const Row & r)\n{\n" + statements(e, ks.value) + "    return n" + std::to_string(ks.value_node) + ";\n}\n";
+    std::vector<char> fcols(ks.live.col.size()), vcols(ks.live.col.size());
+    for (size_t j = 0; j < ks.live.col.size(); ++j)
+        fcols[j] = ks.filter_col(j), vcols[j] = ks.value_only(j);
+    auto vec_loads = [&](const std::vector<char> & which, const char * name, const std::string & indent, const std::string & cond) {
+        std::string t;
+        for (size_t j = 0; j < which.size(); ++j)
+            if (which[j])
+            {
+                const std::string ty = vtype(e->input_types[j]), J = std::to_string(j);
+                t += "#pragma unroll\n" + indent + "for (int k = 0; k < " + std::to_string(JIT_UNROLL) + "; ++k) " + cond + name + J +
+                     "[k] = __builtin_nontemporal_load((const " + ty + " *)a.in[" + J + "] + vb + (u64)k * 64);\n";
+            }
+        return t;
+    };
+    auto vec_decls = [&](const std::vector<char> & which, const char * name, const std::string & U) {
+        std::string t;
+        for (size_t j = 0; j < which.size(); ++j)
+            if (which[j])
+                t += "        " + vtype(e->input_types[j]) + " " + name + std::to_string(j) + "[" + U + "];\n";
+        return t;
+    };
+    auto row_from = [&](const std::vector<char> & which, const char * name) {
+        std::string t;
+        for (size_t j = 0; j < which.size(); ++j)
+            if (which[j])
+                t += "                r.c" + std::to_string(j) + " = " + name + std::to_string(j) + "[k][q];\n";
+        return t;
+    };
+    const std::string U = std::to_string(JIT_UNROLL), VS = std::to_string(V);
+    const std::string unroll_k = "#pragma unroll\n        for (int k = 0; k < " + U + "; ++k)\n";
+    const std::string unroll_q = "#pragma unroll\n            for (int q = 0; q < " + VS + "; ++q)\n";
+    s += "extern \"C\" __global__ __launch_bounds__(256) void k_run(Args a)\n{\n    u64 acc = 0; u64 cnt = 0;\n";
+    s += "    const u64 nvec = a.n / " + VS + ";\n    constexpr u64 CH = 256ull * " + U + ";\n    const u64 nch = nvec / CH;\n";
+    s += "    for (u64 ch = blockIdx.x; ch < nch; ch += gridDim.x)\n    {\n        const u64 sb = ch * CH + (u64)(threadIdx.x >> 6) * (64 * " + U +
+         ");\n        const u64 vb = sb + (threadIdx.x & 63);\n";
+    s += vec_decls(fcols, "x", U) + vec_decls(vcols, "y", U) + "        u32 m[" + U + "];\n";
+    s += vec_loads(fcols, "x", "        ", "");
+    s += unroll_k + "        {\n            u32 mk = 0;\n" + unroll_q + "            {\n                Row r;\n" + row_from(fcols, "x") +
+         "                mk |= eval_keep(r) ? 1u << q : 0u;\n            }\n            m[k] = mk;\n            cnt += (u32)__popc(mk);\n        }\n";
+    s += vec_loads(vcols, "y", "        ", "if (m[k]) ");
+    s += unroll_k + "        {\n            if (m[k])\n            {\n" + unroll_q + "            {\n                Row r;\n" + row_from(fcols, "x") + row_from(vcols, "y") +
+         "                acc += (m[k] >> q) & 1u ? (u64)eval_val(r) : 0ull;\n            }\n            }\n        }\n    }\n";
+    s += "    for (u64 i = nch * CH * " + VS + " + (u64)blockIdx.x * 256 + threadIdx.x; i < a.n; i += (u64)gridDim.x * 256)\n    {\n        Row r;\n";
+    s += row_load(e, fcols, "        ", "i") + "        const bool keep = eval_keep(r);\n        cnt += keep ? 1u : 0u;\n        if (keep)\n        {\n";
+    s += row_load(e, vcols, "            ", "i") + "            acc += (u64)eval_val(r);\n        }\n    }\n";
+    return sum_finish(s, false);
 }
 
 constexpr u32 FE_CHUNK = 1024;
 
 std::string gen_filter_source(const chgpu_expr * e, const KernelSpec & ks)
 {
-    std::string s = gen_frame(e, "", true, ks.filter_node, out_fields(e, ks.out_nodes));
-    const std::string load = row_load(e, "            ", "in ? i : 0");
+    std::string s = gen_frame(e, ks.live, "", true, ks.filter_node, out_fields(e, ks.out_nodes));
+    const std::string load = row_load(e, ks.live.col,"            ", "in ? i : 0");
     const std::string C = std::to_string(FE_CHUNK);
     s += "extern \"C\" __global__ __launch_bounds__(256) void k_fcount(Args a)\n{\n"
          "    const u32 lane = threadIdx.x & 63;\n"
@@ -674,11 +791,11 @@
     return s;
 }
 
-std::string gen_minmax_source(const chgpu_expr * e, int filter_node, int value_node)
+std::string gen_minmax_source(const chgpu_expr * e, const Deps & live, int filter_node, int value_node)
 {
     const std::string v = "n" + std::to_string(value_node);
     const std::string key = chgpu_type_is_signed(e->types[value_node]) ? "(u64)(i64)" + v + " ^ 0x8000000000000000ull" : "(u64)" + v;
-    std::string s = gen_frame(e, "", true, filter_node, {{"u64", "key", key}});
+    std::string s = gen_frame(e, live, "", true, filter_node, {{"u64", "key", key}});
     s += R"SRC(
 DEV u64 shfl_u64(u64 v, int d) { return ((u64)__shfl_down((u32)(v >> 32), d, 64) << 32) | __shfl_down((u32)v, d, 64); }
 extern "C" __global__ __launch_bounds__(256) void k_mm(Args a)
@@ -693,7 +810,7 @@
             const u64 i = i0 + (u64)q * stride;
             const bool in = i < a.n;
             Row r; Res o;
-)SRC" + row_load(e, "            ", "in ? i : 0") + R"SRC(
+)SRC" + row_load(e, live.col, "            ", "in ? i : 0") + R"SRC(
             eval(r, o);
             if (in && o.keep) { lo = o.key < lo ? o.key : lo; hi = o.key > hi ? o.key : hi; ++cnt; }
         }
@@ -713,16 +830,28 @@
         a.part[3 * blockIdx.x] = lo; a.part[3 * blockIdx.x + 1] = hi; a.part[3 * blockIdx.x + 2] = cnt;
     }
 }
-extern "C" __global__ __launch_bounds__(64) void k_mm_fin(Args a)
-{
-    if (threadIdx.x != 0) return;
+extern "C" __global__ __launch_bounds__(256) void k_mm_fin(Args a)
+{
+    constexpr u32 BATCH = 2048; // as k_fin: the partials through LDS, 48 KiB a turn, folded by one lane
+    __shared__ u64 sp[3 * BATCH];
     u64 lo = ~0ull, hi = 0ull, cnt = 0;
-    for (u32 p = 0; p < a.n_parts; ++p)
-    {
-        const u64 l2 = a.part[3 * p], h2 = a.part[3 * p + 1];
-        lo = l2 < lo ? l2 : lo; hi = h2 > hi ? h2 : hi; cnt += a.part[3 * p + 2];
-    }
-    a.part[3 * a.n_parts] = lo; a.part[3 * a.n_parts + 1] = hi; a.part[3 * a.n_parts + 2] = cnt;
+    for (u32 p0 = 0; p0 < a.n_parts; p0 += BATCH)
+    {
+        const u32 m = a.n_parts - p0 < BATCH ? a.n_parts - p0 : BATCH;
+        for (u32 i = threadIdx.x; i < 3 * m; i += 256) sp[i] = a.part[3 * (u64)p0 + i];
+        __syncthreads();
+        if (threadIdx.x == 0)
+        {
+#pragma unroll 8
+            for (u32 p = 0; p < m; ++p)
+            {
+                const u64 l2 = sp[3 * p], h2 = sp[3 * p + 1];
+                lo = l2 < lo ? l2 : lo; hi = h2 > hi ? h2 : hi; cnt += sp[3 * p + 2];
+            }
+        }
+        __syncthreads();
+    }
+    if (threadIdx.x == 0) { a.part[3 * a.n_parts] = lo; a.part[3 * a.n_parts + 1] = hi; a.part[3 * a.n_parts + 2] = cnt; }
 }
 )SRC";
     return s;
@@ -735,6 +864,9 @@
     if (it == g_code_cache.end())
     {
         CHGPU_TRY(rtc_load());
+        if (const char * dump = getenv("CHGPU_JIT_DUMP"))
+            if (strcmp(dump, "all") == 0)
+                fprintf(stderr, "%s\n", src.c_str());
         void * prog = nullptr;
         if (g_rtc.create(&prog, src.c_str(), "chgpu_expr.hip", 0, nullptr, nullptr) != 0)
             return chgpu_set_error(CHGPU_ERR_DEVICE, "hiprtcCreateProgram failed");
@@ -780,80 +912,93 @@
     return CHGPU_OK;
 }
 
-int check_spec(const chgpu_expr * e, uint32_t n_cols, const chgpu_col * const * cols, u64 * rows_out)
-{
-    CHGPU_REQUIRE(n_cols >= e->input_types.size(), CHGPU_ERR_BAD_ARGUMENTS, "expression reads column %zu, %u columns given", e->input_types.size() - 1, n_cols);
+int check_filter_node(const chgpu_expr * e, int filter_node, bool required)
+{
+    CHGPU_REQUIRE(filter_node < (int)e->types.size() && (filter_node >= 0 || !required), CHGPU_ERR_BAD_ARGUMENTS, "bad node");
+    CHGPU_REQUIRE(filter_node < 0 || chgpu_type_is_int(e->types[filter_node]), CHGPU_ERR_BAD_ARGUMENTS,
+                  "Illegal type for filter: the WHERE node must be an integer (FilterDescription.cpp:86-92)");
+    return CHGPU_OK;
+}
+
+int make_spec(const chgpu_expr * e, Form form, uint32_t n_outputs, const uint32_t * out_nodes, int filter_node, int value_node, KernelSpec * ks)
+{
+    ks->form = form;
+    std::vector<int> roots;
+    if (form == FORM_SUM)
+    {
+        CHGPU_REQUIRE(value_node < (int)e->types.size(), CHGPU_ERR_BAD_ARGUMENTS, "bad node");
+        ks->value_node = value_node;
+        roots.push_back(value_node);
+    }
+    else
+    {
+        const uint32_t most = form == FORM_WHERE_MAP ? JIT_MAX_COLS - 1 : JIT_MAX_COLS;
+        CHGPU_REQUIRE(n_outputs > 0 && n_outputs <= most && out_nodes, CHGPU_ERR_BAD_ARGUMENTS, "1..%u outputs", most);
+        for (uint32_t o = 0; o < n_outputs; ++o)
+        {
+            CHGPU_REQUIRE(out_nodes[o] < e->types.size(), CHGPU_ERR_BAD_ARGUMENTS, "bad output node");
+            ks->out_nodes.push_back(out_nodes[o]);
+            roots.push_back((int)out_nodes[o]);
+        }
+    }
+    if (form != FORM_MAP)
+    {
+        CHGPU_TRY(check_filter_node(e, filter_node, form == FORM_WHERE_MAP));
+        ks->filter_node = filter_node;
+    }
+    ks->filter = closure(e, {ks->filter_node});
+    ks->value = closure(e, roots);
+    ks->live = ks->filter | ks->value;
+    std::vector<int> touched;
+    for (size_t j = 0; j < ks->live.col.size(); ++j)
+        if (ks->live.col[j])
+            touched.push_back(e->input_types[j]);
+    for (u32 o : ks->out_nodes)
+        touched.push_back(e->types[o]);
+    ks->vec = vec_rows(touched);
+    return CHGPU_OK;
+}
+
+int check_spec(const chgpu_expr * e, const Deps & live, uint32_t n_cols, const chgpu_col * const * cols, u64 * rows_out)
+{
     u64 rows = 0;
     bool first = true;
     for (size_t j = 0; j < e->input_types.size(); ++j)
     {
         if (e->input_types[j] < 0)
             continue;
-        CHGPU_REQUIRE(cols[j], CHGPU_ERR_BAD_ARGUMENTS, "column %zu is NULL", j);
-        CHGPU_REQUIRE(cols[j]->type == e->input_types[j], CHGPU_ERR_BAD_ARGUMENTS, "column %zu has type %d, the expression was compiled for %d", j, cols[j]->type, e->input_types[j]);
+        const chgpu_col * c = j < n_cols ? cols[j] : nullptr;
+        if (live.col[j])
+        {
+            CHGPU_REQUIRE(j < n_cols, CHGPU_ERR_BAD_ARGUMENTS, "expression reads column %zu, %u columns given", j, n_cols);
+            CHGPU_REQUIRE(c, CHGPU_ERR_BAD_ARGUMENTS, "column %zu is NULL", j);
+        }
+        if (!c)
+            continue;
+        CHGPU_REQUIRE(c->type == e->input_types[j], CHGPU_ERR_BAD_ARGUMENTS, "column %zu has type %d, the expression was compiled for %d", j, c->type, e->input_types[j]);
         if (first)
-            rows = cols[j]->rows, first = false;
-        CHGPU_REQUIRE(cols[j]->rows == rows, CHGPU_ERR_SIZES_MISMATCH, "Sizes of columns doesn't match: %llu and %llu", (unsigned long long)cols[j]->rows, (unsigned long long)rows);
+            rows = c->rows, first = false;
+        CHGPU_REQUIRE(c->rows == rows, CHGPU_ERR_SIZES_MISMATCH, "Sizes of columns doesn't match: %llu and %llu", (unsigned long long)c->rows, (unsigned long long)rows);
     }
     CHGPU_REQUIRE(!first, CHGPU_ERR_BAD_ARGUMENTS, "an expression without input columns has no row count");
     *rows_out = rows;
     return CHGPU_OK;
 }
 
-int check_filter_node(const chgpu_expr * e, int filter_node, bool required)
-{
-    CHGPU_REQUIRE(filter_node < (int)e->types.size() && (filter_node >= 0 || !required), CHGPU_ERR_BAD_ARGUMENTS, "bad node");
-    CHGPU_REQUIRE(filter_node < 0 || chgpu_type_is_int(e->types[filter_node]), CHGPU_ERR_BAD_ARGUMENTS,
-                  "Illegal type for filter: the WHERE node must be an integer (FilterDescription.cpp:86-92)");
-    return CHGPU_OK;
-}
-
-int make_spec(const chgpu_expr * e, Form form, uint32_t n_outputs, const uint32_t * out_nodes, int filter_node, int value_node, bool aligned, KernelSpec * ks)
-{
-    ks->form = form;
-    std::vector<int> touched;
-    for (int t : e->input_types)
-        if (t >= 0)
-            touched.push_back(t);
-    if (form == FORM_SUM)
-    {
-        CHGPU_REQUIRE(value_node < (int)e->types.size(), CHGPU_ERR_BAD_ARGUMENTS, "bad node");
-        ks->value_node = value_node;
-    }
-    else
-    {
-        const uint32_t most = form == FORM_WHERE_MAP ? JIT_MAX_COLS - 1 : JIT_MAX_COLS;
-        CHGPU_REQUIRE(n_outputs > 0 && n_outputs <= most && out_nodes, CHGPU_ERR_BAD_ARGUMENTS, "1..%u outputs", most);
-        for (uint32_t o = 0; o < n_outputs; ++o)
-        {
-            CHGPU_REQUIRE(out_nodes[o] < e->types.size(), CHGPU_ERR_BAD_ARGUMENTS, "bad output node");
-            ks->out_nodes.push_back(out_nodes[o]);
-            touched.push_back(e->types[out_nodes[o]]);
-        }
-    }
-    if (form != FORM_MAP)
-    {
-        CHGPU_TRY(check_filter_node(e, filter_node, form == FORM_WHERE_MAP));
-        ks->filter_node = filter_node;
-    }
-    ks->vec = aligned ? vec_rows(touched) : 1;
-    return CHGPU_OK;
-}
-
-bool cols_aligned(const chgpu_expr * e, const chgpu_col * const * cols)
-{
-    for (size_t j = 0; j < e->input_types.size(); ++j)
-        if (e->input_types[j] >= 0 && ((uintptr_t)cols[j]->data & 63) != 0)
+bool cols_aligned(const Deps & live, const chgpu_col * const * cols)
+{
+    for (size_t j = 0; j < live.col.size(); ++j)
+        if (live.col[j] && ((uintptr_t)cols[j]->data & 63) != 0)
             return false;
     return true;
 }
 
-JitArgs bind_inputs(const chgpu_expr * e, const chgpu_col * const * cols, u64 rows)
+JitArgs bind_inputs(const Deps & live, const chgpu_col * const * cols, u64 rows)
 {
     JitArgs a;
     memset(&a, 0, sizeof(a));
-    for (size_t j = 0; j < e->input_types.size(); ++j)
-        a.in[j] = e->input_types[j] >= 0 ? cols[j]->data : nullptr;
+    for (size_t j = 0; j < live.col.size(); ++j)
+        a.in[j] = live.col[j] ? cols[j]->data : nullptr;
     a.n = rows;
     return a;
 }
@@ -884,7 +1029,7 @@
     return (rows + ks.vec * JIT_UNROLL - 1) / (ks.vec * JIT_UNROLL);
 }
 
-int run_reduction(chgpu_ctx * ctx, const chgpu_expr * e, const chgpu_col * const * cols, u64 rows, const std::string & src, const char * kernel,
+int run_reduction(chgpu_ctx * ctx, const Deps & live, const chgpu_col * const * cols, u64 rows, const std::string & src, const char * kernel,
                   const char * fin, u64 items, int wg_per_cu, u32 words, u64 * res)
 {
     hipFunction_t fn = nullptr, ffin = nullptr;
@@ -892,11 +1037,11 @@
     const u32 grid = chgpu_grid_for(ctx, items, 256, wg_per_cu);
     void * scratch = nullptr;
     CHGPU_TRY(chgpu_scratch(ctx, ((size_t)grid + 1) * words * sizeof(u64), &scratch));
-    JitArgs a = bind_inputs(e, cols, rows);
+    JitArgs a = bind_inputs(live, cols, rows);
     a.part = (u64 *)scratch;
     a.n_parts = grid;
     CHGPU_TRY(launch(ctx, fn, grid, 256, a));
-    CHGPU_TRY(launch(ctx, ffin, 1, 64, a));
+    CHGPU_TRY(launch(ctx, ffin, 1, FIN_THREADS, a));
     ctx->counters[6] += 2;
     return chgpu_read_back(ctx, a.part + (size_t)words * grid, res, words * sizeof(u64));
 }
@@ -926,6 +1071,27 @@
         cols.clear();
     }
 };
+
+bool lazy_applies(const chgpu_expr * e, const KernelSpec & ks)
+{
+    if (ks.form != FORM_SUM || ks.filter_node < 0 || ks.value_node < 0 || ks.vec <= 1 || !chgpu_type_is_int(e->types[ks.value_node]))
+        return false;
+    for (size_t j = 0; j < ks.live.col.size(); ++j)
+        if (ks.value_only(j))
+            return true;
+    return false;
+}
+size_t narrowest_value_only(const chgpu_expr * e, const KernelSpec & ks)
+{
+    size_t w = 8;
+    for (size_t j = 0; j < ks.live.col.size(); ++j)
+        if (ks.value_only(j))
+            w = std::min(w, chgpu_type_size(e->input_types[j]));
+    return w;
+}
+double touched_share(double p, size_t w) { return 1.0 - pow(1.0 - p, 128.0 / (double)w); }
+constexpr double JIT_LAZY_F = 0.48;
+constexpr int JIT_WG_SUM_LAZY = 4;
 
 }
 
@@ -1014,9 +1180,10 @@
 {
     CHGPU_REQUIRE(e, CHGPU_ERR_BAD_ARGUMENTS, "NULL argument");
     KernelSpec ks;
-    CHGPU_TRY(make_spec(e, n_outputs == 0 ? FORM_SUM : filter_node >= 0 ? FORM_WHERE_MAP : FORM_MAP, n_outputs, out_nodes, filter_node, value_node, true, &ks));
+    CHGPU_TRY(make_spec(e, n_outputs == 0 ? FORM_SUM : filter_node >= 0 ? FORM_WHERE_MAP : FORM_MAP, n_outputs, out_nodes, filter_node, value_node, &ks));
+    ks.lazy = lazy_applies(e, ks) && jit_env(nullptr, "tune_jit_lazy", -1) == 1;
     const std::vector<char> * code = nullptr;
-    CHGPU_TRY(jit_compile(ks.form == FORM_WHERE_MAP ? gen_filter_source(e, ks) : gen_source(e, ks), &code));
+    CHGPU_TRY(jit_compile(ks.form == FORM_WHERE_MAP ? gen_filter_source(e, ks) : ks.lazy ? gen_lazy_sum_source(e, ks) : gen_source(e, ks), &code));
     if (code_bytes_out)
         *code_bytes_out = code->size();
     return CHGPU_OK;
@@ -1027,13 +1194,15 @@
 {
     ChgpuDeviceGuard _dev_guard(ctx);
     CHGPU_REQUIRE(ctx && e && cols && outs, CHGPU_ERR_BAD_ARGUMENTS, "NULL argument");
+    KernelSpec ks;
+    CHGPU_TRY(make_spec(e, FORM_MAP, n_outputs, out_nodes, -1, -1, &ks));
     u64 rows = 0;
-    CHGPU_TRY(check_spec(e, n_cols, cols, &rows));
-    KernelSpec ks;
-    CHGPU_TRY(make_spec(e, FORM_MAP, n_outputs, out_nodes, -1, -1, cols_aligned(e, cols), &ks));
+    CHGPU_TRY(check_spec(e, ks.live, n_cols, cols, &rows));
+    if (!cols_aligned(ks.live, cols))
+        ks.vec = 1;
     hipFunction_t fn = nullptr;
     CHGPU_TRY(jit_functions(ctx, gen_source(e, ks), {{"k_run", &fn}}));
-    JitArgs a = bind_inputs(e, cols, rows);
+    JitArgs a = bind_inputs(ks.live, cols, rows);
     OutCols res;
     CHGPU_TRY(res.alloc(ctx, e, ks.out_nodes, rows, a));
     if (rows)
@@ -1050,15 +1219,34 @@
 {
     ChgpuDeviceGuard _dev_guard(ctx);
     CHGPU_REQUIRE(ctx && e && cols, CHGPU_ERR_BAD_ARGUMENTS, "NULL argument");
+    KernelSpec ks;
+    CHGPU_TRY(make_spec(e, FORM_SUM, 0, nullptr, filter_node, value_node, &ks));
     u64 rows = 0;
-    CHGPU_TRY(check_spec(e, n_cols, cols, &rows));
-    KernelSpec ks;
-    CHGPU_TRY(make_spec(e, FORM_SUM, 0, nullptr, filter_node, value_node, cols_aligned(e, cols), &ks));
+    CHGPU_TRY(check_spec(e, ks.live, n_cols, cols, &rows));
+    if (!cols_aligned(ks.live, cols))
+        ks.vec = 1;
     if (result_type_out)
         *result_type_out = value_node >= 0 ? chgpu_sum_result_type(e->types[value_node]) : CHGPU_U64;
     u64 res[2] = {0, 0};
     if (rows)
-        CHGPU_TRY(run_reduction(ctx, e, cols, rows, gen_source(e, ks), "k_run", "k_fin", run_items(rows, ks), jit_env(ctx, "tune_jit_wg_sum", 2), 2, res));
+    {
+        const int mode = lazy_applies(e, ks) ? jit_env(ctx, "tune_jit_lazy", -1) : 0;
+        const std::string lazy_src = mode != 0 ? gen_lazy_sum_source(e, ks) : std::string();
+        if (mode == 1)
+            ks.lazy = true;
+        else if (mode != 0)
+        {
+            auto it = ctx->jit_pass_rate.find(lazy_src);
+            ks.lazy = it != ctx->jit_pass_rate.end() && touched_share(it->second, narrowest_value_only(e, ks)) < JIT_LAZY_F;
+        }
+        if (jit_env(ctx, "debug", 0))
+            fprintf(stderr, "chgpu_expr_filter_sum_node: %s k_run\n", ks.lazy ? "lazy" : "eager");
+        const int wg_eager = jit_env(ctx, "tune_jit_wg_sum", 2);
+        const int wg = ks.lazy ? jit_env(ctx, "tune_jit_wg_sum", JIT_WG_SUM_LAZY) : wg_eager;
+        CHGPU_TRY(run_reduction(ctx, ks.live, cols, rows, ks.lazy ? lazy_src : gen_source(e, ks), "k_run", "k_fin", run_items(rows, ks), wg, 2, res));
+        if (mode != 0 && rows >= (u64)256 * JIT_UNROLL * ks.vec)
+            ctx->jit_pass_rate[lazy_src] = (double)res[1] / (double)rows;
+    }
     if (sum_out)
         memcpy(sum_out, &res[0], 8);
     if (count_out)
@@ -1072,10 +1260,10 @@
     ChgpuDeviceGuard _dev_guard(ctx);
     CHGPU_REQUIRE(ctx && e && cols && outs && rows_out && out_nodes, CHGPU_ERR_BAD_ARGUMENTS, "NULL argument");
     KernelSpec ks;
-    CHGPU_TRY(make_spec(e, FORM_WHERE_MAP, n_outputs, out_nodes, (int)filter_node, -1, false, &ks));
+    CHGPU_TRY(make_spec(e, FORM_WHERE_MAP, n_outputs, out_nodes, (int)filter_node, -1, &ks));
     u64 rows = 0;
-    CHGPU_TRY(check_spec(e, n_cols, cols, &rows));
-    JitArgs a = bind_inputs(e, cols, rows);
+    CHGPU_TRY(check_spec(e, ks.live, n_cols, cols, &rows));
+    JitArgs a = bind_inputs(ks.live, cols, rows);
     OutCols res;
     u64 total = 0;
     if (rows)
@@ -1122,13 +1310,14 @@
     const int vt = e->types[value_node];
     CHGPU_REQUIRE(chgpu_type_is_int(vt), CHGPU_ERR_NOT_IMPLEMENTED,
                   "min / max of a Float column keep a NaN that arrives first (SingleValueDataFixed::setIfSmaller): order-dependent, CPU path");
+    const Deps live = closure(e, {filter_node, (int)value_node});
     u64 rows = 0;
-    CHGPU_TRY(check_spec(e, n_cols, cols, &rows));
+    CHGPU_TRY(check_spec(e, live, n_cols, cols, &rows));
     if (value_type_out)
         *value_type_out = vt;
     u64 res[3] = {~0ull, 0, 0};
     if (rows)
-        CHGPU_TRY(run_reduction(ctx, e, cols, rows, gen_minmax_source(e, filter_node, (int)value_node), "k_mm", "k_mm_fin", (rows + 3) / 4, 8, 3, res));
+        CHGPU_TRY(run_reduction(ctx, live, cols, rows, gen_minmax_source(e, live, filter_node, (int)value_node), "k_mm", "k_mm_fin", (rows + 3) / 4, 8, 3, res));
     const u64 sign = chgpu_type_is_signed(vt) ? 0x8000000000000000ull : 0;
     const u64 vmin = res[2] ? (res[0] ^ sign) : 0, vmax = res[2] ? (res[1] ^ sign) : 0;
     const size_t es = chgpu_type_size(vt);
```

Result: no change. 893.9 billion rows/s (-0.0%).
